# NVlabs/CenterPose

Hardware: NVIDIA H100
Metric: images/sec at 512x512 DLA-34 (dla_34 + DCNv2, 7 heads, decode + PnP) (higher is better)
Workload: dtype tf32x3

## Files before the change

### centerpose_b200/_lib.py

```python
import ctypes
import os

HERE = os.path.dirname(os.path.abspath(__file__))
LIB_PATH = os.environ.get("CP_LIB_PATH") or os.path.join(HERE, "libcenterpose_b200.so")

CP_MAX_HEADS = 16
CP_POSE_RECORD = 192
CP_DETS_RECORD = 128
CP_META_DOUBLES = 16
CP_MAX_K = 128
CP_MAX_MODELS = 16

CP_ARCH_DLA34 = 0
CP_ARCH_DLAV1_34 = 1
CP_ARCH_RES_18, CP_ARCH_RES_34, CP_ARCH_RES_50, CP_ARCH_RES_101, CP_ARCH_RES_152 = 2, 3, 4, 5, 6
CP_PREC_FP32 = 0
CP_PREC_TF32X3 = 1
CP_PREC_BF16 = 2
CP_PREC_TF32 = 3
PRECISIONS = {"fp32": CP_PREC_FP32, "tf32x3": CP_PREC_TF32X3, "bf16": CP_PREC_BF16, "tf32": CP_PREC_TF32}

P_SCORE, P_CLS, P_STATUS, P_NPTS, P_BBOX, P_CT, P_KPS = 0, 1, 2, 3, 4, 8, 10
P_KPS_DISP_MEAN, P_KPS_HM_MEAN, P_KPS_HM_STD, P_KPS_HM_HEIGHT, P_KPS_DISP_STD = 26, 42, 58, 74, 82
P_OBJ_SCALE, P_OBJ_SCALE_UNC, P_TRACKING, P_TRACKING_HP = 98, 101, 104, 106
P_LOCATION, P_QUAT, P_REPROJ, P_PROJ_CUBOID, P_KPS_3D_CAM, P_KPS_PNP, P_SRC_INDEX = 122, 125, 129, 130, 146, 173, 191
D_BBOX, D_SCORE, D_CLS, D_KPS, D_OBJ_SCALE, D_OBJ_SCALE_UNC, D_TRACKING, D_TRACKING_HP = 0, 4, 5, 6, 22, 25, 28, 30
D_KPS_DISP_MEAN, D_KPS_DISP_STD, D_KPS_HM_MEAN, D_KPS_HM_STD, D_KPS_HM_HEIGHT, D_IND = 46, 62, 78, 94, 110, 118
CP_TRACK_RECORD = 320
T_ID, T_AGE, T_ACTIVE, T_IN_BOXES, T_PNP2_STATUS, T_CONF_AVG = 192, 193, 194, 195, 196, 197
T_KPS_FUSION_MEAN, T_KPS_FUSION_STD, T_KPS_MEAN_KF, T_KPS_STD_KF = 200, 216, 232, 248
T_OBJ_SCALE_KF, T_OBJ_SCALE_UNC_KF, T_KPS_PNP_KF, T_KPS_3D_CAM_KF = 264, 267, 270, 288
CP_SEED_RECORD = 264
S_KPS_FUSION_MEAN, S_KPS_FUSION_STD, S_KPS_GT, S_HAS_CT, S_HAS_KPS_GT, S_KPS_PNP_KF, S_HAS_KPS_PNP_KF = 192, 208, 224, 242, 243, 244, 262
RENDER_TRACKS, RENDER_GT, RENDER_EMPTY = 0, 1, 2
PNP_NOT_RUN, PNP_OK, PNP_INVISIBLE, PNP_BEHIND, PNP_FEW_POINTS, PNP_SOLVER_FAIL = 0, 1, 2, 3, 4, 5

EXPORTS = [
    "cp_version", "cp_last_error", "cp_plan_create", "cp_plan_destroy", "cp_plan_load_weights",
    "cp_forward", "cp_plan_bytes", "cp_plan_forward_launches", "cp_decode_workspace_bytes",
    "cp_decode_pnp", "cp_infer", "cp_dcn_v2_forward", "cp_preprocess", "cp_plan_num_ops", "cp_plan_profile",
    "cp_dcn_v2_forward_ex", "cp_conv2d", "cp_dcn_v2_backward",
    "cp_preprocess_affine", "cp_tracker_create", "cp_tracker_destroy", "cp_tracker_reset", "cp_tracker_step", "cp_tracker_render",
    "cp_tracker_render_ex", "cp_tracker_seed", "cp_plan_op_desc", "cp_plan_arena", "cp_plan_run_ops",
    "cp_preprocess_ragged", "cp_tracker_step_ex", "cp_tracker_render_ex2", "cp_tracker_seed_ex",
    "cp_plan_create_multi", "cp_plan_load_weights_model", "cp_plan_num_models", "cp_plan_op_desc_model", "cp_infer_multi",
    "cp_plan_create_multi_track", "cp_infer_multi_track", "cp_tracker_create_multi",
    "cp_plan_create_ex", "cp_plan_memory", "cp_plan_allocations", "cp_preprocess_yuv420",
]

CP_PIX_NV12, CP_PIX_I420 = 0, 1
PIXEL_FORMATS = ("bgr", "nv12", "i420")

CP_PLAN_REUSE_ACTIVATIONS = 1
CP_PLAN_MULTI_TRACK = 2

FAM_NONE, FAM_IGEMM_FP32, FAM_STEM, FAM_CONV3_C16, FAM_IGEMM_UMMA, FAM_CONV_TMA, FAM_DCN_TMA = 0, 1, 2, 3, 4, 5, 6
FAM_MAXPOOL, FAM_UPADD, FAM_GN_RELU, FAM_GRU = 7, 8, 9, 10
FAMILY_NAMES = {FAM_NONE: "fused", FAM_IGEMM_FP32: "igemm_fp32", FAM_STEM: "stem", FAM_CONV3_C16: "conv3_c16",
                FAM_IGEMM_UMMA: "igemm_umma", FAM_CONV_TMA: "conv_tma", FAM_DCN_TMA: "dcn_tma", FAM_MAXPOOL: "maxpool",
                FAM_UPADD: "upadd", FAM_GN_RELU: "gn_relu", FAM_GRU: "gru"}


class CpOpStat(ctypes.Structure):
    _fields_ = [("name", ctypes.c_char * 96), ("kind", ctypes.c_int32), ("ms", ctypes.c_float),
                ("flops", ctypes.c_double), ("bytes", ctypes.c_double)]


class CpActDesc(ctypes.Structure):
    _fields_ = [("off", ctypes.c_int64), ("ext", ctypes.c_int32), ("C", ctypes.c_int32), ("H", ctypes.c_int32),
                ("W", ctypes.c_int32), ("stride", ctypes.c_int32)]


class CpOpDesc(ctypes.Structure):
    _fields_ = ([("name", ctypes.c_char * 96)] +
                [(n, ctypes.c_int32) for n in ("kind", "family", "x3", "nsrc")] +
                [("src", CpActDesc * 4), ("out", CpActDesc), ("out_head", ctypes.c_int32)] +
                [(n, ctypes.c_int32) for n in ("kh", "stride", "pad", "Cin", "Cout", "CoutPad", "Kpad")] +
                [("w", ctypes.c_void_p), ("w_ld", ctypes.c_int32), ("bias", ctypes.c_void_p)] +
                [(n, ctypes.c_int32) for n in ("relu", "has_res", "res_after_relu")] +
                [("res", CpActDesc), ("om", CpActDesc), ("up_w", ctypes.c_void_p), ("f", ctypes.c_int32),
                 ("has_skip", ctypes.c_int32), ("skip", CpActDesc), ("gamma", ctypes.c_void_p),
                 ("beta", ctypes.c_void_p), ("groups", ctypes.c_int32), ("gx", CpActDesc), ("gh", CpActDesc),
                 ("gprev", CpActDesc), ("first_step", ctypes.c_int32)] +
                [(n, ctypes.c_int32) for n in ("fuse_heads", "fused_away", "parent", "n_children")] +
                [("children", ctypes.c_int32 * CP_MAX_HEADS)])


class CpOpLaunch(ctypes.Structure):
    _fields_ = [(n, ctypes.c_int32) for n in ("family", "BN", "ksplit", "grid")]


class CpMemoryInfo(ctypes.Structure):
    _fields_ = [(n, ctypes.c_int64) for n in ("activation_bytes", "weight_bytes", "tile_bytes", "workspace_bytes")]


class CpActAlloc(ctypes.Structure):
    _fields_ = [("floats", ctypes.c_int64), ("off", ctypes.c_int64), ("first", ctypes.c_int32), ("last", ctypes.c_int32)]


class CpConfig(ctypes.Structure):
    _fields_ = [
        ("arch", ctypes.c_int32), ("tracking", ctypes.c_int32), ("tracking_task_gru", ctypes.c_int32),
        ("max_batch", ctypes.c_int32), ("height", ctypes.c_int32), ("width", ctypes.c_int32),
        ("precision", ctypes.c_int32), ("device", ctypes.c_int32), ("head_conv", ctypes.c_int32),
        ("num_heads", ctypes.c_int32),
        ("head_names", ctypes.c_char_p * CP_MAX_HEADS),
        ("head_channels", ctypes.c_int32 * CP_MAX_HEADS),
    ]


class CpHeads(ctypes.Structure):
    _fields_ = [(n, ctypes.c_void_p) for n in (
        "hm", "wh", "hps", "reg", "hm_hp", "hp_offset", "scale", "hps_uncertainty",
        "scale_uncertainty", "tracking", "tracking_hp")]


class CpDecodeParams(ctypes.Structure):
    _fields_ = [
        ("batch", ctypes.c_int32), ("out_h", ctypes.c_int32), ("out_w", ctypes.c_int32),
        ("num_classes", ctypes.c_int32), ("num_joints", ctypes.c_int32), ("K", ctypes.c_int32),
        ("rep_mode", ctypes.c_int32), ("use_moments", ctypes.c_int32), ("nms", ctypes.c_int32),
        ("visible_thresh", ctypes.c_int32), ("opencv_return", ctypes.c_int32),
        ("apply_sigmoid", ctypes.c_int32), ("use_pnp", ctypes.c_int32),
        ("vis_thresh", ctypes.c_float), ("balance", ctypes.c_float), ("modern_bool_semantics", ctypes.c_int32),
        ("test_scale", ctypes.c_float), ("num_scales", ctypes.c_int32),
    ]


class CpTrackerConfig(ctypes.Structure):
    _fields_ = [(n, ctypes.c_int32) for n in (
        "streams", "max_tracks", "kalman", "scale_pool", "use_pnp", "hps_uncertainty", "max_age", "visible_thresh",
        "opencv_return", "render_hm_mode", "render_hmhp_mode", "device")] + [
        (n, ctypes.c_float) for n in ("new_thresh", "pre_thresh", "R", "conf_lo", "conf_hi")] + [
        ("hungarian", ctypes.c_int32)]


_lib = None


def lib_available():
    return os.path.exists(LIB_PATH)


def load():
    global _lib
    if _lib is not None:
        return _lib
    if not os.path.exists(LIB_PATH):
        raise RuntimeError(
            "centerpose_b200: %s not found -- run `python -m centerpose_b200.build` "
            "(there is no CPU / PyTorch fallback for the hot path)" % LIB_PATH)
    L = ctypes.CDLL(LIB_PATH)
    vp, i32, i64 = ctypes.c_void_p, ctypes.c_int32, ctypes.c_int64
    L.cp_version.restype = ctypes.c_int
    L.cp_last_error.restype = ctypes.c_char_p
    L.cp_plan_create.argtypes = [ctypes.POINTER(CpConfig), ctypes.POINTER(vp)]
    L.cp_plan_destroy.argtypes = [vp]
    L.cp_plan_load_weights.argtypes = [vp, ctypes.POINTER(ctypes.c_char_p), ctypes.POINTER(vp),
                                       ctypes.POINTER(i64), i32, vp]
    L.cp_forward.argtypes = [vp, i32, vp, vp, vp, vp, ctypes.POINTER(vp), vp]
    L.cp_plan_num_ops.argtypes = [vp]
    L.cp_plan_profile.argtypes = [vp, i32, vp, vp, vp, vp, ctypes.POINTER(vp), vp, ctypes.POINTER(CpOpStat), i32,
                                  ctypes.POINTER(i32)]
    L.cp_plan_op_desc.argtypes = [vp, i32, ctypes.POINTER(CpOpDesc)]
    L.cp_plan_arena.argtypes = [vp, ctypes.POINTER(vp), ctypes.POINTER(i64)]
    L.cp_plan_run_ops.argtypes = [vp, i32, i32, i32, vp, vp, vp, vp, ctypes.POINTER(vp), vp, ctypes.POINTER(CpOpLaunch)]
    L.cp_plan_bytes.argtypes = [vp]
    L.cp_plan_bytes.restype = i64
    L.cp_plan_forward_launches.argtypes = [vp]
    L.cp_plan_forward_launches.restype = i32
    L.cp_decode_workspace_bytes.argtypes = [ctypes.POINTER(CpDecodeParams)]
    L.cp_decode_workspace_bytes.restype = ctypes.c_size_t
    L.cp_decode_pnp.argtypes = [ctypes.POINTER(CpDecodeParams), ctypes.POINTER(CpHeads), vp, vp, vp, vp, vp,
                                ctypes.c_size_t, vp]
    L.cp_infer.argtypes = [vp, i32, vp, vp, vp, vp, ctypes.POINTER(CpDecodeParams), vp,
                           ctypes.POINTER(vp), vp, vp, vp, vp]
    L.cp_dcn_v2_forward.argtypes = [vp, vp, vp, vp, vp, vp, i32, i32, i32, i32, i32, vp]
    L.cp_dcn_v2_forward_ex.argtypes = [vp, vp, vp, vp, vp, vp, i32, i32, i32, i32, i32, i32, vp]
    L.cp_dcn_v2_backward.argtypes = [vp] * 10 + [i32] * 6 + [vp]
    L.cp_conv2d.argtypes = [vp, vp, vp, vp, vp, i32, i32, i32, i32, i32, i32, i32, i32, i32, i32, vp]
    L.cp_preprocess.argtypes = [vp, vp, i32, i32, i32, i32, i32, ctypes.POINTER(ctypes.c_float),
                                ctypes.POINTER(ctypes.c_float), vp]
    L.cp_preprocess_affine.argtypes = [vp, vp, i32, i32, i32, i32, i32, ctypes.POINTER(ctypes.c_double),
                                       ctypes.POINTER(ctypes.c_float), ctypes.POINTER(ctypes.c_float), vp]
    L.cp_preprocess_ragged.argtypes = [vp, i64, ctypes.POINTER(i64), ctypes.POINTER(i32), vp, i32, i32, i32,
                                       ctypes.POINTER(ctypes.c_double), ctypes.POINTER(ctypes.c_float),
                                       ctypes.POINTER(ctypes.c_float), vp]
    L.cp_preprocess_yuv420.argtypes = [vp, i64, ctypes.POINTER(i64), ctypes.POINTER(i32), i32, vp, i32, i32, i32,
                                       ctypes.POINTER(ctypes.c_double), ctypes.POINTER(ctypes.c_float),
                                       ctypes.POINTER(ctypes.c_float), vp]
    L.cp_tracker_create.argtypes = [ctypes.POINTER(CpTrackerConfig), ctypes.POINTER(vp)]
    L.cp_tracker_destroy.argtypes = [vp]
    L.cp_tracker_reset.argtypes = [vp, i32, vp]
    L.cp_tracker_step.argtypes = [vp, i32, vp, vp, i32, vp, vp, vp, vp]
    L.cp_tracker_render.argtypes = [vp, i32, vp, vp, i32, i32, vp, vp, vp]
    L.cp_tracker_render_ex.argtypes = [vp, i32, vp, vp, i32, i32, ctypes.POINTER(i32), vp, vp, vp]
    L.cp_tracker_seed.argtypes = [vp, i32, vp, vp, i32, vp]
    L.cp_tracker_step_ex.argtypes = [vp, i32, ctypes.POINTER(i32), vp, vp, i32, vp, vp, vp, vp]
    L.cp_tracker_render_ex2.argtypes = [vp, i32, ctypes.POINTER(i32), vp, vp, i32, i32, ctypes.POINTER(i32), vp, vp, vp]
    L.cp_tracker_seed_ex.argtypes = [vp, i32, ctypes.POINTER(i32), vp, vp, i32, vp]
    L.cp_plan_create_multi.argtypes = [ctypes.POINTER(CpConfig), i32, ctypes.POINTER(vp)]
    L.cp_plan_load_weights_model.argtypes = [vp, i32, ctypes.POINTER(ctypes.c_char_p), ctypes.POINTER(vp),
                                             ctypes.POINTER(i64), i32, vp]
    L.cp_plan_num_models.argtypes = [vp]
    L.cp_plan_op_desc_model.argtypes = [vp, i32, i32, ctypes.POINTER(CpOpDesc)]
    L.cp_infer_multi.argtypes = [vp, i32, vp, ctypes.POINTER(CpDecodeParams), vp, ctypes.POINTER(vp), vp, vp, vp, vp]
    L.cp_plan_create_multi_track.argtypes = [ctypes.POINTER(CpConfig), i32, ctypes.POINTER(vp)]
    L.cp_infer_multi_track.argtypes = [vp, i32, vp, vp, vp, vp, ctypes.POINTER(CpDecodeParams), vp, ctypes.POINTER(vp), vp,
                                       vp, vp, vp]
    L.cp_tracker_create_multi.argtypes = [ctypes.POINTER(CpTrackerConfig), i32, ctypes.POINTER(vp)]
    L.cp_plan_create_ex.argtypes = [ctypes.POINTER(CpConfig), i32, ctypes.c_uint32, ctypes.POINTER(vp)]
    L.cp_plan_memory.argtypes = [ctypes.POINTER(CpConfig), i32, ctypes.c_uint32, ctypes.POINTER(CpMemoryInfo)]
    L.cp_plan_allocations.argtypes = [ctypes.POINTER(CpConfig), i32, ctypes.c_uint32, ctypes.POINTER(CpActAlloc), i32,
                                      ctypes.POINTER(i32)]
    for name in EXPORTS:
        fn = getattr(L, name)
        if name not in ("cp_version", "cp_last_error", "cp_plan_bytes", "cp_plan_forward_launches",
                        "cp_decode_workspace_bytes"):
            fn.restype = ctypes.c_int
    _lib = L
    return L


def check(rc, what=""):
    if rc != 0:
        msg = load().cp_last_error()
        raise RuntimeError("centerpose_b200 %s failed (%d): %s" % (what, rc, msg.decode() if msg else "?"))
```

### centerpose_b200/csrc/common.cuh

```cuda
#pragma once
#include <cuda_runtime.h>
#include <stdint.h>
#include <stdio.h>
#include <string>

#include "../../include/centerpose_b200.h"

namespace cp {

void set_error(const std::string& msg);
int fail(int code, const std::string& msg);
extern thread_local long long g_launch_counter;

#define CP_CUDA_CHECK(expr)                                                              \
  do {                                                                                   \
    cudaError_t _e = (expr);                                                             \
    if (_e != cudaSuccess)                                                               \
      return ::cp::fail(CP_ERR_CUDA, std::string(#expr) + ": " + cudaGetErrorString(_e)); \
  } while (0)

#define CP_LAUNCH_CHECK(what)                                                            \
  do {                                                                                   \
    cudaError_t _e = cudaGetLastError();                                                 \
    if (_e != cudaSuccess)                                                               \
      return ::cp::fail(CP_ERR_CUDA, std::string(what) + ": " + cudaGetErrorString(_e));  \
    ++::cp::g_launch_counter;                                                            \
  } while (0)

enum IgemmMode {
  IGEMM_NCHW_SCALAR = 0,
  IGEMM_NHWC_VEC = 1,
  IGEMM_DCN = 2,
  IGEMM_DECONV = 3
};
__host__ __device__ __forceinline__ int deconv_dy(int p, int a) { return p ? 1 - a : -a; }
__host__ __device__ __forceinline__ int deconv_ky(int p, int a) { return p ? 2 * a : 1 + 2 * a; }

struct IgemmParams {
  const float* src[4];
  int srcC[4];
  int srcStride[4];
  int nsrc;
  int B, Hin, Win, Cin;
  int Hout, Wout, Cout, CoutPad;
  int kh, kw, stride, pad;
  int Kpad;
  const float* wgt;
  const float* bias;
  const float* residual;
  int resStride;
  int relu;
  int res_after_relu;
  float* out;
  int outStride;
  int out_nchw;
  const float* offmask;
  int omStride;
  int mask_is_logit;
  int mode;
  const void* wgt_umma;
  float* splitk_ws;
  size_t splitk_ws_floats;
  int fuse_n, fuse_hidden;
  const float* fuse_w[16];
  const float* fuse_b[16];
  float* fuse_out[16];
  int fuse_cout[16];
  int ipm;
  long long wstride, tstride;
  unsigned nchw_per_model;
};
inline int model_ipm(const IgemmParams& p) { return p.ipm > 0 ? p.ipm : p.B; }

int launch_igemm_fp32(const IgemmParams& p, cudaStream_t stream);

int decode_pnp_models(const cp_decode_params* prm, int models, const cp_heads* heads, const double* meta, float* dets,
                      float* poses, int32_t* n_valid, void* workspace, size_t workspace_bytes, void* stream);

struct LaunchInfo {
  int BN = 0;
  int ksplit = 1;
  long long grid = 0;
};

bool conv3_c16_supported(const IgemmParams& p);
int launch_conv3_c16(const IgemmParams& p, cudaStream_t stream);
bool stem_supported(const IgemmParams& p);
int launch_stem_conv(const IgemmParams& p, cudaStream_t s);

struct ConvKernel {
  int family = CP_FAM_IGEMM_FP32;
  bool x3 = false;
  bool round_out = false;
  int BN = 0;
  int cslab = 0;
  size_t wbytes = 0;
};
struct ConvPolicy {
  bool small_on_cuda_cores;
  bool dcn_tma;
  bool round_out;
  bool cuda_core_fallback;
};
inline bool known_precision(int32_t precision) {
  return precision == CP_PREC_FP32 || precision == CP_PREC_TF32X3 || precision == CP_PREC_BF16 || precision == CP_PREC_TF32;
}
inline bool gather_x3(int32_t precision) { return precision == CP_PREC_TF32 || precision == CP_PREC_TF32X3; }
ConvKernel select_conv_kernel(const IgemmParams& p, int32_t precision, const ConvPolicy& pol);
struct alignas(64) TmaMaps {
  unsigned char map[4][128];
};
int conv_encode(const ConvKernel& k, const IgemmParams& p, int Bmax, TmaMaps* maps);
int conv_pack(const ConvKernel& k, const IgemmParams& p, int ld, void* tiles, cudaStream_t s);
int conv_launch(const ConvKernel& k, const IgemmParams& p, const TmaMaps* maps, cudaStream_t s, LaunchInfo* info = nullptr);
int run_conv(IgemmParams& p, int32_t precision, const ConvPolicy& pol, cudaStream_t s);

int splitk_factor(long long tiles, int slabs, int num_sms, size_t tile_floats, size_t ws_floats);

bool umma_supported(const IgemmParams& p, int prec);
int umma_tile_n(int CoutPad, int prec);
size_t umma_weight_bytes(int Kreal, int CoutPad, int prec);
int launch_pack_umma_weight(const float* src_k_by_ld, int ld, int Kreal, int Cout, int CoutPad, int prec, void* dst,
                            cudaStream_t s);
int launch_igemm_umma(const IgemmParams& p, int prec, cudaStream_t stream, LaunchInfo* info = nullptr);

int launch_maxpool2(const float* in, float* out, int B, int H, int W, int C, cudaStream_t s);
int launch_maxpool3s2(const float* in, const float* residual, float* out, int B, int H, int W, int C, cudaStream_t s);
int launch_pack_deconv_weight(const float* w_io44, const float* scale, float* out, int Cin, int Cout, int CoutPad, int Kpad,
                              cudaStream_t s);
int launch_upsample_add(const float* in, const float* wgt_kkc, const float* skip, float* out, int B,
                        int Hin, int Win, int C, int f, cudaStream_t s, int ipm = 0, long long wstride = 0);
int launch_pack_conv_weight(const float* w_oihw, const float* scale, float* out, int Cout, int Cin,
                            int kh, int kw, int CoutPad, int Kpad, int ld, int colOff, cudaStream_t s,
                            int CinPad = 0);
int launch_pack_bias(const float* conv_bias, const float* bn_w, const float* bn_b, const float* bn_mean,
                     const float* bn_var, float* scale_out, float* bias_out, int C, int CPad, float eps,
                     cudaStream_t s);
int launch_pack_up_weight(const float* w_c1kk, float* out_kkc, int C, int k, cudaStream_t s);
int launch_nchw_to_nhwc(const float* in, float* out, int B, int C, int H, int W, int outStride,
                        int chanOffset, cudaStream_t s);
int launch_nhwc_to_nchw(const float* in, float* out, int B, int C, int H, int W, int inStride, cudaStream_t s);
constexpr int kGnBlocks = 64, kGnMaxGroups = 64;
inline size_t gn_workspace_doubles(int B) { return (size_t)B * kGnMaxGroups * 2 * (1 + kGnBlocks); }
int launch_group_norm_relu(float* x, const float* gamma, const float* beta, int B, int HW, int C,
                           int stride, int chanOffset, int groups, float eps, double* ws, cudaStream_t s, int ipm = 0,
                           long long wstride = 0);
int launch_gru_gates(const float* xi, const float* hh, const float* hprev, float* hout, int B_HW, int C,
                     int first_step, cudaStream_t s);

constexpr int kX3GroupBlocks = 1;

bool tma_conv_supported(const IgemmParams& p, int x3);
size_t tma_weight_bytes(int Cin, int taps, int CoutPad, int x3);
int tma_tile_n(int CoutPad, int x3);
int tma_cslab(const IgemmParams& p, int x3);
int launch_pack_tma_weight(const float* src_k_by_ld, int ld, int Cin, int taps, int Cout, int CoutPad, int x3, int cslab,
                           int bn, void* dst, cudaStream_t s);
int tma_encode_nhwc_box(const float* base, int C, int W, int H, int B, int strideFloats, int boxC, int boxW, int boxH,
                        int swizzle64, void* map_out );
int tma_conv_encode(const IgemmParams& p, int Bmax, int cslab, void* maps_out );
int launch_conv_tma(const IgemmParams& p, const void* maps, const ConvKernel& k, cudaStream_t stream, LaunchInfo* info);

bool dcn_tma_supported(const IgemmParams& p, int x3);
int dcn_tma_tile_n(int CoutPad, int x3);
int dcn_tma_encode(const IgemmParams& p, int Bmax, void* map_out );
int launch_dcn_tma(const IgemmParams& p, const void* map, const ConvKernel& k, cudaStream_t stream, LaunchInfo* info);

inline int round_up(int x, int m) { return (x + m - 1) / m * m; }
inline int conv_cout_pad(int Cout) { return round_up(Cout, Cout > 32 ? 64 : (Cout > 16 ? 32 : 16)); }

extern thread_local int g_pdl;
#ifdef __CUDACC__
__device__ __forceinline__ void griddep_wait() { asm volatile("griddepcontrol.wait;" ::: "memory"); }
__device__ __forceinline__ void griddep_launch_dependents() { asm volatile("griddepcontrol.launch_dependents;" ::: "memory"); }
template <typename... KArgs, typename... Args>
inline cudaError_t launch_kernel(void (*kern)(KArgs...), dim3 grid, dim3 block, size_t smem, cudaStream_t s, Args&&... args) {
  cudaLaunchConfig_t cfg{};
  cfg.gridDim = grid;
  cfg.blockDim = block;
  cfg.dynamicSmemBytes = smem;
  cfg.stream = s;
  cudaLaunchAttribute attr[1];
  attr[0].id = cudaLaunchAttributeProgrammaticStreamSerialization;
  attr[0].val.programmaticStreamSerializationAllowed = 1;
  cfg.attrs = attr;
  cfg.numAttrs = g_pdl ? 1 : 0;
  return cudaLaunchKernelEx(&cfg, kern, static_cast<KArgs>(args)...);
}
#endif
constexpr size_t kSplitkWsFloats = (size_t)160 * 256 * 128;

constexpr int kMaxDevices = 64;
inline int current_device_slot() {
  int d = 0;
  if (cudaGetDevice(&d) != cudaSuccess || d < 0 || d >= kMaxDevices) d = 0;
  return d;
}
template <typename T, int N = 1>
struct PerDevice {
  T v[kMaxDevices][N] = {};
  T& here(int slot = 0) { return v[current_device_slot()][slot]; }
};
inline int device_sm_count(int* out) {
  static PerDevice<int> cache;
  int& n = cache.here();
  if (!n) {
    int dev = 0;
    CP_CUDA_CHECK(cudaGetDevice(&dev));
    CP_CUDA_CHECK(cudaDeviceGetAttribute(&n, cudaDevAttrMultiProcessorCount, dev));
  }
  *out = n;
  return CP_OK;
}

}
```

### centerpose_b200/csrc/conv_select.cu

```cuda
#include <stdlib.h>

#include "common.cuh"

namespace cp {

ConvKernel select_conv_kernel(const IgemmParams& p, int32_t precision, const ConvPolicy& pol) {
  const bool small = p.mode == IGEMM_NCHW_SCALAR || p.Cin < 32;
  if (precision != CP_PREC_FP32 && !(pol.small_on_cuda_cores && small)) {
    const bool tma = precision == CP_PREC_TF32 || precision == CP_PREC_TF32X3;
    const bool x3 = precision == CP_PREC_TF32X3;
    if (tma && pol.dcn_tma && dcn_tma_supported(p, x3))
      return {CP_FAM_DCN_TMA, x3, pol.round_out && !x3, dcn_tma_tile_n(p.CoutPad, x3), 16,
              tma_weight_bytes(p.Cin, 9, p.CoutPad, x3)};
    if (tma && tma_conv_supported(p, x3))
      return {CP_FAM_CONV_TMA, x3, pol.round_out && !x3, tma_tile_n(p.CoutPad, x3), tma_cslab(p, x3),
              tma_weight_bytes(p.Cin, p.kh * p.kw, p.CoutPad, x3)};
    const bool gx3 = gather_x3(precision);
    const int phases = p.mode == IGEMM_DECONV ? 4 : 1;
    if (umma_supported(p, gx3))
      return {CP_FAM_IGEMM_UMMA, gx3, false, umma_tile_n(p.CoutPad, gx3), 0,
              phases * umma_weight_bytes(p.kh * p.kw * p.Cin, p.CoutPad, gx3)};
    if (!pol.cuda_core_fallback) return {CP_FAM_NONE};
  }
  return {stem_supported(p) ? CP_FAM_STEM : (conv3_c16_supported(p) ? CP_FAM_CONV3_C16 : CP_FAM_IGEMM_FP32)};
}

int conv_encode(const ConvKernel& k, const IgemmParams& p, int Bmax, TmaMaps* maps) {
  if (k.family == CP_FAM_DCN_TMA) return dcn_tma_encode(p, Bmax, maps->map);
  if (k.family == CP_FAM_CONV_TMA) return tma_conv_encode(p, Bmax, k.cslab, maps->map);
  return CP_OK;
}

int conv_pack(const ConvKernel& k, const IgemmParams& p, int ld, void* tiles, cudaStream_t s) {
  switch (k.family) {
    case CP_FAM_DCN_TMA:
    case CP_FAM_CONV_TMA:
      return launch_pack_tma_weight(p.wgt, ld, p.Cin, p.kh * p.kw, p.Cout, p.CoutPad, k.x3, k.cslab, k.BN, tiles, s);
    case CP_FAM_IGEMM_UMMA: {
      const int phases = p.mode == IGEMM_DECONV ? 4 : 1;
      const size_t phase_bytes = k.wbytes / phases;
      for (int ph = 0; ph < phases; ++ph)
        if (int rc = launch_pack_umma_weight(p.wgt + (size_t)ph * p.Kpad * ld, ld, p.kh * p.kw * p.Cin, p.Cout, p.CoutPad,
                                             k.x3, (unsigned char*)tiles + ph * phase_bytes, s))
          return rc;
      return CP_OK;
    }
    default:
      return CP_OK;
  }
}

int conv_launch(const ConvKernel& k, const IgemmParams& p, const TmaMaps* maps, cudaStream_t s, LaunchInfo* info) {
  switch (k.family) {
    case CP_FAM_DCN_TMA: return launch_dcn_tma(p, maps->map, k, s, info);
    case CP_FAM_CONV_TMA: return launch_conv_tma(p, maps->map, k, s, info);
    case CP_FAM_IGEMM_UMMA: return launch_igemm_umma(p, k.x3, s, info);
    case CP_FAM_STEM: return launch_stem_conv(p, s);
    case CP_FAM_CONV3_C16: return launch_conv3_c16(p, s);
    case CP_FAM_IGEMM_FP32: return launch_igemm_fp32(p, s);
    default: return fail(CP_ERR_INVALID, "conv: no kernel selected");
  }
}

int run_conv(IgemmParams& p, int32_t precision, const ConvPolicy& pol, cudaStream_t s) {
  const ConvKernel k = select_conv_kernel(p, precision, pol);
  if (k.family == CP_FAM_NONE) return fail(CP_ERR_INVALID, "shape not supported by the wgmma kernel");
  if (!k.wbytes) return conv_launch(k, p, nullptr, s);
  void* tiles = nullptr;
  CP_CUDA_CHECK(cudaMallocAsync(&tiles, k.wbytes, s));
  TmaMaps maps;
  int rc = conv_encode(k, p, p.B, &maps);
  if (!rc) rc = conv_pack(k, p, p.CoutPad, tiles, s);
  if (!rc) {
    p.wgt_umma = tiles;
    rc = conv_launch(k, p, &maps, s);
  }
  cudaFreeAsync(tiles, s);
  return rc;
}

int splitk_factor(long long tiles, int slabs, int num_sms, size_t tile_floats, size_t ws_floats) {
  const char* off = getenv("CP_NO_SPLITK");
  if (!ws_floats || (off && atoi(off) != 0)) return 1;
  int S = 1;
  for (int cand = 2; cand <= slabs; ++cand)
    if (slabs % cand == 0 && tiles * cand <= num_sms && (size_t)tiles * cand * tile_floats <= ws_floats) S = cand;
  return S;
}

}
```

### centerpose_b200/csrc/conv_tma.cu

```cuda
#include <cuda.h>

#include "common.cuh"
#include "umma_common.cuh"

namespace cp {
namespace {

constexpr int TM_BM = 128;
constexpr int TM_THREADS = 384;
constexpr int TM_THREADS_X3 = 512;

struct TmaConvParams {
  CUtensorMap amap[4];
  int nsrc;
  int srcC[4];
  int B, H, W, Cin, Cout, CoutPad, BN;
  int k;
  int tile_m;
  int Wt, boxh;
  int tiles_per_image;
  long long total_tiles;
  long long m_tiles;
  uint32_t slab_bytes, slab_stride;
  int SA, SB;
  const float* bias;
  const float* residual;
  int resStride, relu, res_after_relu;
  float* out;
  int outStride, out_nchw;
  int round_tf32;
  int cslab;
  int x3;
  int group;
  const unsigned char* wtiles;
  int ksplit, sps;
  float* part;
  int fuse, tph;
  const float* fuse_w[16];
  const float* fuse_b[16];
  float* fuse_out[16];
  int fuse_cout[16];
  int ipm;
  long long wstride, tstride, tiles_per_model;
};

using namespace umma;

struct TmaCtl {
  unsigned long long a_full[4], a_empty[4], a_split[4];
  unsigned long long b_full[8], b_empty[8];
};
static_assert(sizeof(TmaCtl) <= 512, "control block");

struct TileGeo {
  int n_tile, img, g0, r_lo, model;
  long long pos0;
};
template <bool MULTI>
__device__ __forceinline__ TileGeo decode_tile(const TmaConvParams& p, long long ct, int n_tiles) {
  TileGeo g;
  g.n_tile = (int)(ct % n_tiles);
  const long long m_tile = ct / n_tiles;
  g.img = 0;
  g.g0 = 0;
  g.r_lo = 0;
  g.pos0 = 0;
  g.model = 0;
  if (p.k == 3) {
    g.img = (int)(m_tile / p.tiles_per_image);
    g.g0 = (int)(m_tile - (long long)g.img * p.tiles_per_image) * p.tile_m;
    const int t = g.g0 - 1;
    g.r_lo = (t >= 0) ? t / p.Wt : -((-t + p.Wt - 1) / p.Wt);
    if (MULTI) g.model = g.img / p.ipm;
  } else if (MULTI) {
    g.model = (int)(m_tile / p.tiles_per_model);
    g.pos0 = (long long)g.model * p.ipm * p.H * p.W + (m_tile - g.model * p.tiles_per_model) * p.tile_m;
  } else {
    g.pos0 = m_tile * p.tile_m;
  }
  return g;
}

template <bool MULTI>
__device__ __forceinline__ bool tile_position(const TmaConvParams& p, const TileGeo& g, int i, int* n, int* oy, int* ox, int* m) {
  bool valid;
  if (p.k == 3) {
    const int gg = g.g0 + i;
    *oy = gg / p.Wt;
    const int xp = gg - *oy * p.Wt;
    *ox = xp - 1;
    *n = g.img;
    valid = (*oy < p.H) && (xp >= 1) && (xp <= p.W);
  } else {
    const long long pix = g.pos0 + i;
    valid = pix < (MULTI ? (long long)(g.model + 1) * p.ipm : (long long)p.B) * p.H * p.W;
    const long long pp = valid ? pix : 0;
    *ox = (int)(pp % p.W);
    const long long t = pp / p.W;
    *oy = (int)(t % p.H);
    *n = (int)(t / p.H);
  }
  *m = (int)(((size_t)*n * p.H + *oy) * p.W + *ox);
  return valid;
}

template <bool X3, bool FUSE, int BN, bool MULTI>
__global__ void __launch_bounds__(X3 ? TM_THREADS_X3 : TM_THREADS, 1) conv_tma_kernel(const __grid_constant__ TmaConvParams p) {
  extern __shared__ __align__(1024) unsigned char smem[];
  TmaCtl* ctl = reinterpret_cast<TmaCtl*>(smem);
  if (threadIdx.x == 0) griddep_launch_dependents();
  const uint32_t slabs0 = (smem_u32(smem) + 512u + 1023u) & ~1023u;
  const uint32_t rowb = (uint32_t)p.cslab * 4u;
  const uint32_t btile_bytes = (uint32_t)BN * rowb * (X3 ? 2u : 1u);
  const uint32_t a_stage = p.slab_stride * (X3 ? 2u : 1u);
  const uint32_t btiles0 = slabs0 + (uint32_t)p.SA * a_stage;
  const uint32_t drain0 = btiles0 + (uint32_t)p.SB * btile_bytes;

  const int tid = threadIdx.x, warp = tid >> 5, lane = tid & 31;
  const int n_tiles = p.CoutPad / BN;
  const int taps = p.k * p.k;
  const int KS_SPLIT = p.ksplit;
  const int sps = p.sps;
  const int KB = sps * taps;
  const int KB_all = (p.Cin / p.cslab) * taps;
  const long long total_tiles = p.total_tiles;
  const long long tph = FUSE ? p.tph : 1;
  auto tile_at = [&](long long it) { return ((long long)blockIdx.x + (it / tph) * gridDim.x) * tph + (it % tph); };

  if (tid == 0) {
    for (int s = 0; s < p.SA; ++s) {
      mbar_init(smem_u32(&ctl->a_full[s]), 1);
      mbar_init(smem_u32(&ctl->a_empty[s]), 2);
      mbar_init(smem_u32(&ctl->a_split[s]), 128);
    }
    for (int s = 0; s < p.SB; ++s) {
      mbar_init(smem_u32(&ctl->b_full[s]), 1);
      mbar_init(smem_u32(&ctl->b_empty[s]), 2);
    }
    fence_mbar_init();
  }
  __syncthreads();
  if (warp != 1) griddep_wait();

  if (warp < 4) {
    if (X3) asm volatile("setmaxnreg.dec.sync.aligned.u32 40;");
    if (warp == 0) {
      if (lane == 0) {
        int stage = 0;
        uint32_t phase = 0;
        for (long long it = 0, tile = tile_at(0); tile < total_tiles; tile = tile_at(++it)) {
          const TileGeo g = decode_tile<MULTI>(p, tile / KS_SPLIT, n_tiles);
          const int s_begin = (int)(tile % KS_SPLIT) * sps;
          for (int s = s_begin; s < s_begin + sps; ++s) {
            int src = 0, cb = 0;
            while (src + 1 < p.nsrc && s * p.cslab >= cb + p.srcC[src]) {
              cb += p.srcC[src];
              ++src;
            }
            mbar_wait(smem_u32(&ctl->a_empty[stage]), phase ^ 1u);
            const uint32_t bar = smem_u32(&ctl->a_full[stage]);
            mbar_arrive_expect_tx(bar, p.slab_bytes);
            const uint32_t dst = slabs0 + (uint32_t)stage * a_stage;
            if (p.k == 3)
              tma_load_4d(dst, &p.amap[src], s * p.cslab - cb, -1, g.r_lo - 1, g.img, bar);
            else
              tma_load_2d(dst, &p.amap[src], s * p.cslab - cb, (int)g.pos0, bar);
            if (++stage == p.SA) {
              stage = 0;
              phase ^= 1u;
            }
          }
        }
      }
      __syncwarp();
    } else if (warp == 1) {
      if (lane == 0) {
        int stage = 0;
        uint32_t phase = 0;
        for (long long it = 0, tile = tile_at(0); tile < total_tiles; tile = tile_at(++it)) {
          const unsigned char* wsrc;
          if constexpr (MULTI) {
            const TileGeo g = decode_tile<MULTI>(p, tile / KS_SPLIT, n_tiles);
            wsrc = p.wtiles + (size_t)g.model * p.tstride +
                   ((size_t)g.n_tile * KB_all + (size_t)(tile % KS_SPLIT) * KB) * btile_bytes;
          } else {
            const int n_tile = (int)((tile / KS_SPLIT) % n_tiles);
            wsrc = p.wtiles + ((size_t)n_tile * KB_all + (size_t)(tile % KS_SPLIT) * KB) * btile_bytes;
          }
          for (int kb = 0; kb < KB; ++kb) {
            mbar_wait(smem_u32(&ctl->b_empty[stage]), phase ^ 1u);
            const uint32_t bar = smem_u32(&ctl->b_full[stage]);
            mbar_arrive_expect_tx(bar, btile_bytes);
            bulk_g2s(btiles0 + (uint32_t)stage * btile_bytes, wsrc + (size_t)kb * btile_bytes, btile_bytes, bar);
            if (++stage == p.SB) {
              stage = 0;
              phase ^= 1u;
            }
          }
        }
      }
      __syncwarp();
    }
  } else if (X3 && warp >= 12) {
    asm volatile("setmaxnreg.dec.sync.aligned.u32 48;");
    const int st = tid - 384;
    int stage = 0;
    uint32_t phase = 0;
    const uint32_t nchunk = p.slab_bytes >> 4;
    for (long long it = 0, tile = tile_at(0); tile < total_tiles; tile = tile_at(++it)) {
      for (int s = 0; s < sps; ++s) {
        mbar_wait(smem_u32(&ctl->a_full[stage]), phase);
        const uint32_t hi = slabs0 + (uint32_t)stage * a_stage;
        const uint32_t lo = hi + p.slab_stride;
        for (uint32_t c0 = st; c0 < nchunk; c0 += 128 * 4) {
          float4 v[4];
#pragma unroll
          for (int u = 0; u < 4; ++u)
            if (c0 + u * 128 < nchunk) v[u] = ld_shared_v4f(hi + ((c0 + u * 128) << 4));
#pragma unroll
          for (int u = 0; u < 4; ++u) {
            if (c0 + u * 128 < nchunk) {
              float4 h, l;
              h.x = tf32_round(v[u].x); l.x = tf32_round(v[u].x - h.x);
              h.y = tf32_round(v[u].y); l.y = tf32_round(v[u].y - h.y);
              h.z = tf32_round(v[u].z); l.z = tf32_round(v[u].z - h.z);
              h.w = tf32_round(v[u].w); l.w = tf32_round(v[u].w - h.w);
              st_shared_v4f(hi + ((c0 + u * 128) << 4), h.x, h.y, h.z, h.w);
              st_shared_v4f(lo + ((c0 + u * 128) << 4), l.x, l.y, l.z, l.w);
            }
          }
        }
        fence_proxy_async_smem();
        mbar_arrive(smem_u32(&ctl->a_split[stage]));
        if (++stage == p.SA) {
          stage = 0;
          phase ^= 1u;
        }
      }
    }
  } else {
    if (X3) asm volatile("setmaxnreg.inc.sync.aligned.u32 208;");
    const int c = (warp - 4) >> 2, wt = tid & 127;
    float* dstage = reinterpret_cast<float*>(smem + (drain0 - smem_u32(smem))) + (size_t)c * (DRAIN_STAGE_BYTES / 4);
    const uint32_t bar_a = smem_u32(X3 ? &ctl->a_split[0] : &ctl->a_full[0]);
    const uint32_t bar_a_empty = smem_u32(&ctl->a_empty[0]);
    const uint32_t bar_b_full = smem_u32(&ctl->b_full[0]), bar_b_empty = smem_u32(&ctl->b_empty[0]);
    const uint32_t a_lo_u = p.slab_stride >> 4, b_lo_u = ((uint32_t)BN * rowb) >> 4;
    EpiParams ep;
    ep.bias = p.bias;
    ep.residual = p.residual;
    ep.resStride = p.resStride;
    ep.relu = p.relu;
    ep.res_after_relu = p.res_after_relu;
    ep.round_tf32 = p.round_tf32;
    ep.out = p.out;
    ep.outStride = p.outStride;
    ep.out_nchw = p.out_nchw;
    ep.Cout = p.Cout;
    ep.CoutPad = p.CoutPad;
    ep.H = p.H;
    ep.W = p.W;
    int sa = 0, sb = 0;
    uint32_t pa = 0, pb = 0;
    float acc[BN / 2];
    float sums[X3 ? BN / 2 : 1];
    float acc2[FUSE ? 16 : 1];
#pragma unroll
    for (int j = 0; j < BN / 2; ++j) acc[j] = 0.f;
#pragma unroll
    for (int j = 0; j < (FUSE ? 16 : 1); ++j) acc2[j] = 0.f;
    for (long long it = 0, tile = tile_at(0); tile < total_tiles; tile = tile_at(++it)) {
      const TileGeo g = decode_tile<MULTI>(p, tile / KS_SPLIT, n_tiles);
      const uint32_t row0 = (p.k == 3 ? (uint32_t)(g.g0 - 1 - g.r_lo * p.Wt) : 0u) + (uint32_t)c * 64u;
#pragma unroll
      for (int j = 0; j < (X3 ? BN / 2 : 1); ++j) sums[j] = 0.f;
      int kbi = 0, gk = 0;
      for (int s = 0; s < sps; ++s) {
        mbar_wait(bar_a + 8u * (uint32_t)sa, pa);
        const uint32_t a_slab = slabs0 + (uint32_t)sa * a_stage;
        for (int tap = 0; tap < taps; ++tap, ++kbi) {
          const int ky = tap / 3, kx = tap - ky * 3;
          const uint32_t arow = row0 + (p.k == 3 ? (uint32_t)(ky * p.Wt + kx) : 0u);
          mbar_wait(bar_b_full + 8u * (uint32_t)sb, pb);
          const uint64_t da = make_desc(a_slab + arow * rowb, p.cslab);
          const uint64_t db = make_desc(btiles0 + (uint32_t)sb * btile_bytes, p.cslab);
          const bool fresh = X3 ? gk == 0 : kbi == 0;
          if (p.cslab == 32)
            mma_kblock<BN, X3, false, 4>(acc, da, db, a_lo_u, b_lo_u, fresh);
          else
            mma_kblock<BN, X3, false, 2>(acc, da, db, a_lo_u, b_lo_u, fresh);
          if (wt == 0) {
            mbar_arrive(bar_b_empty + 8u * (uint32_t)sb);
            if (tap == taps - 1) mbar_arrive(bar_a_empty + 8u * (uint32_t)sa);
          }
          if (++sb == p.SB) {
            sb = 0;
            pb ^= 1u;
          }
          if (X3) {
            if (gk == p.group - 1 || kbi == KB - 1) {
#pragma unroll
              for (int j = 0; j < (X3 ? BN / 2 : 1); ++j) sums[j] += acc[X3 ? j : 0];
              gk = 0;
            } else {
              ++gk;
            }
          }
        }
        if (++sa == p.SA) {
          sa = 0;
          pa ^= 1u;
        }
      }
      const int r_me = wt >> 1;
      int n, oy, ox, m;
      const bool valid = tile_position<MULTI>(p, g, c * 64 + r_me, &n, &oy, &ox, &m);
      const int col_end = min(p.Cout, (g.n_tile + 1) * BN);
      const int head = FUSE ? g.n_tile / p.tph : 0, part = FUSE ? g.n_tile - head * p.tph : 0;
      const size_t wofs = MULTI ? (size_t)g.model * p.wstride : 0;
      if (MULTI) ep.bias = p.bias + wofs;
      if (FUSE && part == 0) {
#pragma unroll
        for (int j = 0; j < (FUSE ? 16 : 1); ++j) acc2[j] = 0.f;
      }
      auto fn = [&](int r, int cb, float (&v)[16]) {
        if (cb >= BN) return;
        if (!FUSE && KS_SPLIT > 1) {
          const long long mn = tile / KS_SPLIT;
          const int ks = (int)(tile % KS_SPLIT);
          float4* mine = reinterpret_cast<float4*>(p.part) + (((size_t)mn * KS_SPLIT + ks) * (BN >> 2) + (cb >> 2)) * p.tile_m +
                         c * 64 + r;
#pragma unroll
          for (int q = 0; q < 4; ++q) __stcg(mine + (size_t)q * p.tile_m, make_float4(v[4 * q], v[4 * q + 1], v[4 * q + 2], v[4 * q + 3]));
        } else if (FUSE) {
          const float* b1 = p.bias + wofs + (size_t)g.n_tile * BN + cb;
          const float4* w2 = reinterpret_cast<const float4*>(p.fuse_w[head] + wofs) + ((size_t)part * BN + cb) * 4;
#pragma unroll
          for (int q = 0; q < 16; ++q) {
            const float h = fmaxf(v[q] + __ldg(b1 + q), 0.f);
#pragma unroll
            for (int u = 0; u < 4; ++u) {
              const float4 w = __ldg(w2 + q * 4 + u);
              acc2[FUSE ? 4 * u + 0 : 0] = fmaf(h, w.x, acc2[FUSE ? 4 * u + 0 : 0]);
              acc2[FUSE ? 4 * u + 1 : 0] = fmaf(h, w.y, acc2[FUSE ? 4 * u + 1 : 0]);
              acc2[FUSE ? 4 * u + 2 : 0] = fmaf(h, w.z, acc2[FUSE ? 4 * u + 2 : 0]);
              acc2[FUSE ? 4 * u + 3 : 0] = fmaf(h, w.w, acc2[FUSE ? 4 * u + 3 : 0]);
            }
          }
        } else {
          epilogue_row<16>(ep, v, valid, m, n, oy, ox, g.n_tile * BN + cb, col_end);
        }
      };
      if constexpr (X3)
        drain_rows<BN>(sums, dstage, wt, 1 + c, fn);
      else
        drain_rows<BN>(acc, dstage, wt, 1 + c, fn);
      if (FUSE && part == p.tph - 1) {
#pragma unroll
        for (int j = 0; j < (FUSE ? 16 : 1); ++j) acc2[j] += __shfl_xor_sync(0xffffffffu, acc2[j], 1);
        if ((wt & 1) == 0 && valid) {
          const int co = p.fuse_cout[head];
          float* o = p.fuse_out[head] + ((size_t)n * co * p.H + oy) * p.W + ox;
          const size_t plane = (size_t)p.H * p.W;
#pragma unroll
          for (int j = 0; j < 16; ++j)
            if (j < co) o[j * plane] = acc2[FUSE ? j : 0] + __ldg(p.fuse_b[head] + wofs + j);
        }
      }
    }
  }
}

__global__ void pack_tma_weight_kernel(const float* __restrict__ src, int ld, int Cin, int taps, int Cout, int BN, int n_tiles,
                                       int round_tf32, int x3, int cslab, unsigned char* __restrict__ dst) {
  const int KB = (Cin / cslab) * taps;
  const int cpr = cslab / 4;
  const size_t rowb = (size_t)cslab * 4;
  const size_t total = (size_t)n_tiles * KB * BN * cpr;
  for (size_t i = blockIdx.x * (size_t)blockDim.x + threadIdx.x; i < total; i += (size_t)gridDim.x * blockDim.x) {
    const int q = i % cpr;
    size_t t = i / cpr;
    const int nr = t % BN;
    t /= BN;
    const int kb = t % KB;
    const int nt = t / KB;
    const int n = nt * BN + nr;
    const int slab = kb / taps, tap = kb - slab * taps;
    float v[4];
#pragma unroll
    for (int j = 0; j < 4; ++j) {
      const int k = tap * Cin + slab * cslab + q * 4 + j;
      float x = (n < Cout) ? src[(size_t)k * ld + n] : 0.f;
      v[j] = round_tf32 ? tf32_round(x) : x;
    }
    const size_t tile = ((size_t)nt * KB + kb) * (size_t)BN * rowb * (x3 ? 2 : 1);
    const int sw = cslab == 32 ? (nr & 7) : ((nr >> 1) & 3);
    const size_t off = (size_t)nr * rowb + (size_t)((q ^ sw) << 4);
    *reinterpret_cast<float4*>(dst + tile + off) = make_float4(v[0], v[1], v[2], v[3]);
    if (x3) {
      float l[4];
#pragma unroll
      for (int j = 0; j < 4; ++j) {
        const int k = tap * Cin + slab * cslab + q * 4 + j;
        const float x = (n < Cout) ? src[(size_t)k * ld + n] : 0.f;
        l[j] = tf32_round(x - v[j]);
      }
      *reinterpret_cast<float4*>(dst + tile + (size_t)BN * rowb + off) = make_float4(l[0], l[1], l[2], l[3]);
    }
  }
}

typedef CUresult (*EncodeTiledFn)(CUtensorMap*, CUtensorMapDataType, cuuint32_t, void*, const cuuint64_t*, const cuuint64_t*,
                                  const cuuint32_t*, const cuuint32_t*, CUtensorMapInterleave, CUtensorMapSwizzle,
                                  CUtensorMapL2promotion, CUtensorMapFloatOOBfill);

EncodeTiledFn get_encode() {
  static EncodeTiledFn fn = nullptr;
  if (!fn) {
    void* p = nullptr;
    cudaDriverEntryPointQueryResult q;
    if (cudaGetDriverEntryPoint("cuTensorMapEncodeTiled", &p, cudaEnableDefault, &q) == cudaSuccess &&
        q == cudaDriverEntryPointSuccess)
      fn = (EncodeTiledFn)p;
  }
  return fn;
}

}

template <bool MULTI>
__global__ void __launch_bounds__(256) conv_tma_splitk_finish(const __grid_constant__ TmaConvParams p, long long mn_tiles) {
  splitk_finish<MULTI>(p, p.tile_m, mn_tiles, [&](long long mn, int i, int* n, int* oy, int* ox) {
    int m;
    return tile_position<MULTI>(p, decode_tile<MULTI>(p, mn, p.CoutPad / p.BN), i, n, oy, ox, &m);
  });
}

static int tma_boxh(int Wt) { return (TM_BM + 1 + 2 * Wt + Wt - 1) / Wt + 1; }

constexpr size_t TM_BUDGET = 222 * 1024 - 2 * (size_t)DRAIN_STAGE_BYTES;

static int tma_smem_layout(uint32_t a_stage, uint32_t btile, int k, int* SA, int* SB, size_t* smem) {
  const size_t budget = TM_BUDGET;
  int sa = 2;
  if ((size_t)sa * a_stage + 2 * (size_t)btile > budget) sa = 1;
  if ((size_t)sa * a_stage + 2 * (size_t)btile > budget) return fail(CP_ERR_INVALID, "conv_tma: slab does not fit shared memory");
  int sb = (int)((budget - (size_t)sa * a_stage) / btile);
  if (sb > 8) sb = 8;
  if (sb < 2) return fail(CP_ERR_INVALID, "conv_tma: tile does not fit shared memory");
  if (k == 1 && sa < 4) {
    int s4 = (int)((budget - (size_t)sb * btile) / a_stage);
    if (s4 > 4) s4 = 4;
    if (s4 > sa) sa = s4;
  }
  *SA = sa;
  *SB = sb;
  *smem = 512 + 2048 + (size_t)sa * a_stage + (size_t)sb * btile + 2 * (size_t)DRAIN_STAGE_BYTES;
  return CP_OK;
}

int tma_cslab(const IgemmParams& p, int x3) {
  if (p.Cin % 32) return 16;
  if (!x3 || p.kh != 3) return 32;
  const int Wt = p.Win + 2;
  const int boxh = tma_boxh(Wt);
  const size_t slab32 = ((size_t)boxh * Wt * 128 + 1023) / 1024 * 1024;
  const int bn = tma_tile_n(p.CoutPad, x3);
  const size_t need = 2 * (2 * slab32) + 2 * ((size_t)bn * 128 * 2);
  return need > TM_BUDGET ? 16 : 32;
}

int tma_tile_n(int CoutPad, int) { return wgmma_tile_n(CoutPad, 128); }

bool tma_conv_supported(const IgemmParams& p, int x3) {
  if (p.mode != IGEMM_NHWC_VEC) return false;
  if (!((p.kh == 1 && p.kw == 1 && p.pad == 0) || (p.kh == 3 && p.kw == 3 && p.pad == 1))) return false;
  if (p.stride != 1) return false;
  const int cs = tma_cslab(p, x3);
  if (p.Cin % cs) return false;
  for (int s = 0; s < p.nsrc; ++s)
    if (p.srcC[s] % cs || p.srcStride[s] % 4) return false;
  if (p.kh == 3 && p.Win + 2 > 256) return false;
  const int bn = tma_tile_n(p.CoutPad, x3);
  if (bn == 0) return false;
  const size_t slab = p.kh == 3 ? (size_t)tma_boxh(p.Win + 2) * (p.Win + 2) * cs * 4 : (size_t)TM_BM * cs * 4;
  const size_t a_stage = ((slab + 1023) / 1024 * 1024) * (x3 ? 2 : 1);
  const size_t btile = (size_t)bn * cs * 4 * (x3 ? 2 : 1);
  return a_stage + 2 * btile <= TM_BUDGET;
}

size_t tma_weight_bytes(int Cin, int taps, int CoutPad, int x3) {
  return (size_t)CoutPad * Cin * taps * 4 * (x3 ? 2 : 1);
}

int launch_pack_tma_weight(const float* src, int ld, int Cin, int taps, int Cout, int CoutPad, int x3, int cs, int bn,
                           void* dst, cudaStream_t s) {
  const int nt = CoutPad / bn;
  size_t total = (size_t)nt * (Cin / cs) * taps * bn * (cs / 4);
  int blocks = (int)((total + 255) / 256);
  if (blocks > 132 * 32) blocks = 132 * 32;
  pack_tma_weight_kernel<<<blocks, 256, 0, s>>>(src, ld, Cin, taps, Cout, bn, nt, 1, x3, cs, (unsigned char*)dst);
  CP_LAUNCH_CHECK("pack_tma_weight_kernel");
  return CP_OK;
}

int tma_encode_nhwc_box(const float* base, int C, int W, int H, int B, int strideFloats, int boxC, int boxW, int boxH,
                        int swizzle64, void* map_out) {
  EncodeTiledFn enc = get_encode();
  if (!enc) return fail(CP_ERR_CUDA, "cuTensorMapEncodeTiled entry point not available");
  cuuint64_t dims[4] = {(cuuint64_t)C, (cuuint64_t)W, (cuuint64_t)H, (cuuint64_t)B};
  cuuint64_t strides[3] = {(cuuint64_t)strideFloats * 4, (cuuint64_t)W * strideFloats * 4, (cuuint64_t)H * W * strideFloats * 4};
  cuuint32_t box[4] = {(cuuint32_t)boxC, (cuuint32_t)boxW, (cuuint32_t)boxH, 1};
  cuuint32_t es[4] = {1, 1, 1, 1};
  CUresult r = enc(reinterpret_cast<CUtensorMap*>(map_out), CU_TENSOR_MAP_DATA_TYPE_FLOAT32, 4, (void*)base, dims, strides, box,
                   es, CU_TENSOR_MAP_INTERLEAVE_NONE, swizzle64 ? CU_TENSOR_MAP_SWIZZLE_64B : CU_TENSOR_MAP_SWIZZLE_NONE,
                   CU_TENSOR_MAP_L2_PROMOTION_L2_256B,
                   CU_TENSOR_MAP_FLOAT_OOB_FILL_NONE);
  if (r != CUDA_SUCCESS) return fail(CP_ERR_CUDA, "cuTensorMapEncodeTiled failed with code " + std::to_string((int)r));
  return CP_OK;
}

int tma_conv_encode(const IgemmParams& p, int Bmax, int cs, void* maps_out) {
  EncodeTiledFn enc = get_encode();
  if (!enc) return fail(CP_ERR_CUDA, "cuTensorMapEncodeTiled entry point not available");
  CUtensorMap* maps = reinterpret_cast<CUtensorMap*>(maps_out);
  const int Wt = p.Win + 2;
  const int boxh = tma_boxh(Wt);
  const CUtensorMapSwizzle swz = cs == 32 ? CU_TENSOR_MAP_SWIZZLE_128B : CU_TENSOR_MAP_SWIZZLE_64B;
  for (int s = 0; s < p.nsrc; ++s) {
    CUresult r;
    if (p.kh == 3) {
      cuuint64_t dims[4] = {(cuuint64_t)p.srcC[s], (cuuint64_t)p.Win, (cuuint64_t)p.Hin, (cuuint64_t)Bmax};
      cuuint64_t strides[3] = {(cuuint64_t)p.srcStride[s] * 4, (cuuint64_t)p.Win * p.srcStride[s] * 4,
                               (cuuint64_t)p.Hin * p.Win * p.srcStride[s] * 4};
      cuuint32_t box[4] = {(cuuint32_t)cs, (cuuint32_t)Wt, (cuuint32_t)boxh, 1};
      cuuint32_t es[4] = {1, 1, 1, 1};
      r = enc(&maps[s], CU_TENSOR_MAP_DATA_TYPE_FLOAT32, 4, (void*)p.src[s], dims, strides, box, es,
              CU_TENSOR_MAP_INTERLEAVE_NONE, swz, CU_TENSOR_MAP_L2_PROMOTION_L2_256B,
              CU_TENSOR_MAP_FLOAT_OOB_FILL_NONE);
    } else {
      cuuint64_t dims[2] = {(cuuint64_t)p.srcC[s], (cuuint64_t)Bmax * p.Hin * p.Win};
      cuuint64_t strides[1] = {(cuuint64_t)p.srcStride[s] * 4};
      cuuint32_t box[2] = {(cuuint32_t)cs, (cuuint32_t)TM_BM};
      cuuint32_t es[2] = {1, 1};
      r = enc(&maps[s], CU_TENSOR_MAP_DATA_TYPE_FLOAT32, 2, (void*)p.src[s], dims, strides, box, es,
              CU_TENSOR_MAP_INTERLEAVE_NONE, swz, CU_TENSOR_MAP_L2_PROMOTION_L2_256B,
              CU_TENSOR_MAP_FLOAT_OOB_FILL_NONE);
    }
    if (r != CUDA_SUCCESS) return fail(CP_ERR_CUDA, "cuTensorMapEncodeTiled failed with code " + std::to_string((int)r));
  }
  return CP_OK;
}

template <bool X3, bool FUSE, bool MULTI>
static int launch_conv_tma_kernel(const TmaConvParams& q, const cudaLaunchConfig_t& cfg0) {
  void (*kern)(TmaConvParams) = nullptr;
  switch (q.BN) {
    case 16: kern = conv_tma_kernel<X3, FUSE, 16, MULTI>; break;
    case 32: kern = conv_tma_kernel<X3, FUSE, 32, MULTI>; break;
    case 64: kern = conv_tma_kernel<X3, FUSE, 64, MULTI>; break;
    case 128: kern = conv_tma_kernel<X3, FUSE, 128, MULTI>; break;
    default: return fail(CP_ERR_INVALID, "conv_tma: unsupported N tile");
  }
  static PerDevice<bool, 4> configured;
  const int slot = q.BN == 128 ? 3 : (q.BN == 64 ? 2 : (q.BN == 32 ? 1 : 0));
  if (!configured.here(slot)) {
    CP_CUDA_CHECK(cudaFuncSetAttribute(kern, cudaFuncAttributeMaxDynamicSharedMemorySize, 227 * 1024));
    configured.here(slot) = true;
  }
  cudaLaunchConfig_t cfg = cfg0;
  cudaLaunchAttribute attr[1];
  attr[0].id = cudaLaunchAttributeProgrammaticStreamSerialization;
  attr[0].val.programmaticStreamSerializationAllowed = 1;
  cfg.attrs = attr;
  cfg.numAttrs = g_pdl ? 1 : 0;
  CP_CUDA_CHECK(cudaLaunchKernelEx(&cfg, kern, q));
  CP_LAUNCH_CHECK("conv_tma_kernel");
  return CP_OK;
}

int launch_conv_tma(const IgemmParams& p, const void* maps, const ConvKernel& k, cudaStream_t stream, LaunchInfo* info) {
  if (!p.wgt_umma) return fail(CP_ERR_INVALID, "conv_tma: weight tiles missing");
  if (p.B % model_ipm(p)) return fail(CP_ERR_INVALID, "conv_tma: batch is not a whole number of models");
  const bool x3 = k.x3;
  TmaConvParams q;
  memset(&q, 0, sizeof(q));
  memcpy(q.amap, maps, sizeof(CUtensorMap) * 4);
  q.nsrc = p.nsrc;
  for (int s = 0; s < 4; ++s) q.srcC[s] = p.srcC[s];
  q.B = p.B;
  q.H = p.Hin;
  q.W = p.Win;
  q.Cin = p.Cin;
  q.Cout = p.Cout;
  q.CoutPad = p.CoutPad;
  q.BN = k.BN;
  q.x3 = x3;
  q.cslab = k.cslab;
  q.group = kX3GroupBlocks * (32 / q.cslab);
  q.k = p.kh;
  q.Wt = p.Win + 2;
  q.tile_m = TM_BM;
  q.boxh = tma_boxh(q.Wt);
  q.ipm = model_ipm(p);
  q.wstride = p.wstride;
  q.tstride = p.tstride;
  size_t m_tiles;
  if (q.k == 3) {
    q.tiles_per_image = (p.Hin * q.Wt + q.tile_m - 1) / q.tile_m;
    m_tiles = (size_t)q.tiles_per_image * p.B;
    q.slab_bytes = (uint32_t)q.boxh * q.Wt * (uint32_t)q.cslab * 4u;
  } else {
    q.tiles_per_image = 0;
    q.tiles_per_model = ((long long)q.ipm * p.Hin * p.Win + q.tile_m - 1) / q.tile_m;
    m_tiles = (size_t)q.tiles_per_model * (p.B / q.ipm);
    q.slab_bytes = (uint32_t)q.tile_m * (uint32_t)q.cslab * 4u;
  }
  q.slab_stride = (q.slab_bytes + 1023u) & ~1023u;
  const uint32_t btile = (uint32_t)q.BN * (uint32_t)q.cslab * 4u * (x3 ? 2u : 1u);
  const uint32_t a_stage = q.slab_stride * (x3 ? 2u : 1u);
  size_t smem = 0;
  if (int rc = tma_smem_layout(a_stage, btile, q.k, &q.SA, &q.SB, &smem)) return rc;
  q.bias = p.bias;
  q.residual = p.residual;
  q.resStride = p.resStride;
  q.relu = p.relu;
  q.res_after_relu = p.res_after_relu;
  q.out = p.out;
  q.outStride = p.outStride;
  q.out_nchw = p.out_nchw;
  q.round_tf32 = k.round_out;
  q.wtiles = (const unsigned char*)p.wgt_umma;
  if (p.fuse_n > 0) {
    if (p.fuse_hidden % q.BN || p.CoutPad != p.fuse_n * p.fuse_hidden || !p.relu || p.residual || (x3 && q.BN != 128))
      return fail(CP_ERR_INVALID, "conv_tma: fused 1x1 needs relu, no residual and head_conv a multiple of the N tile");
    q.fuse = 1;
    q.tph = p.fuse_hidden / q.BN;
    for (int h = 0; h < p.fuse_n; ++h) {
      q.fuse_w[h] = p.fuse_w[h];
      q.fuse_b[h] = p.fuse_b[h];
      q.fuse_out[h] = p.fuse_out[h];
      q.fuse_cout[h] = p.fuse_cout[h];
    }
  }
  q.m_tiles = (long long)m_tiles;
  q.part = p.splitk_ws;
  const long long mn = (long long)m_tiles * (p.CoutPad / q.BN);
  const int nslab = q.Cin / q.cslab;
  int num_sms = 0;
  if (int rc = device_sm_count(&num_sms)) return rc;
  q.ksplit = x3 && !q.fuse ? splitk_factor(mn, nslab, num_sms, (size_t)q.tile_m * q.BN, p.splitk_ws_floats) : 1;
  q.sps = nslab / q.ksplit;
  q.total_tiles = mn * q.ksplit;
  if (q.total_tiles >= (1ll << 31)) return fail(CP_ERR_INVALID, "conv_tma: too many tiles");
  cudaLaunchConfig_t cfg{};
  cfg.gridDim = dim3((unsigned)(q.total_tiles < num_sms ? q.total_tiles : num_sms));
  cfg.blockDim = dim3(x3 ? TM_THREADS_X3 : TM_THREADS);
  cfg.dynamicSmemBytes = smem;
  cfg.stream = stream;
  const bool multi = p.B > q.ipm;
  int rc;
  if (multi)
    rc = x3 ? (q.fuse ? launch_conv_tma_kernel<true, true, true>(q, cfg) : launch_conv_tma_kernel<true, false, true>(q, cfg))
            : (q.fuse ? launch_conv_tma_kernel<false, true, true>(q, cfg) : launch_conv_tma_kernel<false, false, true>(q, cfg));
  else
    rc = x3 ? (q.fuse ? launch_conv_tma_kernel<true, true, false>(q, cfg) : launch_conv_tma_kernel<true, false, false>(q, cfg))
            : (q.fuse ? launch_conv_tma_kernel<false, true, false>(q, cfg) : launch_conv_tma_kernel<false, false, false>(q, cfg));
  if (rc) return rc;
  if (info) {
    info->BN = q.BN;
    info->ksplit = q.ksplit;
    info->grid = cfg.gridDim.x;
  }
  if (q.ksplit > 1) {
    const long long threads = mn * (q.BN / 4) * q.tile_m;
    CP_CUDA_CHECK(launch_kernel(multi ? conv_tma_splitk_finish<true> : conv_tma_splitk_finish<false>,
                                dim3((unsigned)((threads + 255) / 256)), dim3(256), 0, stream, q, mn));
    CP_LAUNCH_CHECK("conv_tma_splitk_finish");
  }
  return CP_OK;
}

}
```

### centerpose_b200/csrc/dcn_tma.cu

```cuda
#include <cuda.h>

#include "common.cuh"
#include "umma_common.cuh"

namespace cp {
namespace {

using namespace umma;

constexpr int DT_BM = 128;
constexpr int DT_THREADS = 512;
constexpr int DT_CS = 16;
constexpr int DT_PH = 8, DT_PW = 16;
constexpr int DT_HALO = 8;
constexpr int DT_SH = DT_PH + 2 * DT_HALO, DT_SW = DT_PW + 2 * DT_HALO;
constexpr uint32_t DT_SLAB_BYTES = DT_SH * DT_SW * DT_CS * 4;
constexpr uint32_t DT_COEF_BYTES = DT_BM * 9 * 16;

struct DcnTmaParams {
  CUtensorMap amap;
  const float* src;
  int srcStride;
  const float* offmask;
  int omStride, mask_is_logit;
// ... 341 lines not shown
        if (++sb == p.SB) {
          sb = 0;
          pb ^= 1u;
        }
        if (X3) {
          if (gk == p.group - 1 || kbi == KB - 1) {
#pragma unroll
            for (int j = 0; j < (X3 ? BN / 2 : 1); ++j) sums[j] += acc[X3 ? j : 0];
            gk = 0;
          } else {
            ++gk;
          }
        }
      }
      const int n_tile = (int)((tile / KS_SPLIT) % n_tiles);
      const long long m_tile = (tile / KS_SPLIT) / n_tiles;
      const int n = (int)(m_tile / p.tiles_per_image);
      const int pt = (int)(m_tile - (long long)n * p.tiles_per_image);
      const int col_end = min(p.Cout, (n_tile + 1) * BN);
      if (MULTI) ep.bias = p.bias + (size_t)(n / p.ipm) * p.wstride;
      auto fn = [&](int r, int cb0, float (&v)[16]) {
        if (cb0 >= BN) return;
        const int i = c * 64 + r;
        if (KS_SPLIT > 1) {
          float4* part_row = reinterpret_cast<float4*>(p.part) + ((size_t)tile * (BN >> 2) + (cb0 >> 2)) * 128 + i;
#pragma unroll
          for (int q = 0; q < 4; ++q) __stcg(part_row + (size_t)q * 128, make_float4(v[4 * q], v[4 * q + 1], v[4 * q + 2], v[4 * q + 3]));
        } else {
          const int oy = (pt / p.tiles_x) * DT_PH + (i >> 4), ox = (pt % p.tiles_x) * DT_PW + (i & 15);
          const int m = (n * p.H + oy) * p.W + ox;
          epilogue_row<16>(ep, v, true, m, n, oy, ox, n_tile * BN + cb0, col_end);
        }
      };
      if constexpr (X3)
        drain_rows<BN>(sums, dstage, wt, 1 + c, fn);
      else
        drain_rows<BN>(acc, dstage, wt, 1 + c, fn);
    }
  }
}

template <bool MULTI>
__global__ void __launch_bounds__(256) dcn_tma_splitk_finish(const __grid_constant__ DcnTmaParams p, long long mn_tiles) {
  splitk_finish<MULTI>(p, DT_BM, mn_tiles, [&](long long mn, int i, int* n, int* oy, int* ox) {
    const long long m_tile = mn / (p.CoutPad / p.BN);
    *n = (int)(m_tile / p.tiles_per_image);
    const int pt = (int)(m_tile - (long long)*n * p.tiles_per_image);
    *oy = (pt / p.tiles_x) * DT_PH + (i >> 4);
    *ox = (pt % p.tiles_x) * DT_PW + (i & 15);
    return true;
  });
}

}

int dcn_tma_tile_n(int CoutPad, int) { return wgmma_tile_n(CoutPad, 128); }

bool dcn_tma_supported(const IgemmParams& p, int x3) {
  if (p.mode != IGEMM_DCN || p.nsrc != 1) return false;
  if (p.kh != 3 || p.kw != 3 || p.stride != 1 || p.pad != 1) return false;
  if (p.Cin % DT_CS || p.srcStride[0] % 4) return false;
  const int W = p.Win, H = p.Hin;
  if (W > 128 || H > 128 || (W % DT_PW) || (H % DT_PH)) return false;
  return dcn_tma_tile_n(p.CoutPad, x3) != 0;
}

int dcn_tma_encode(const IgemmParams& p, int Bmax, void* map_out) {
  return tma_encode_nhwc_box(p.src[0], p.srcC[0], p.Win, p.Hin, Bmax, p.srcStride[0], DT_CS, DT_SW, DT_SH, 1, map_out);
}

int launch_dcn_tma(const IgemmParams& p, const void* map, const ConvKernel& k, cudaStream_t stream, LaunchInfo* info) {
  const bool x3 = k.x3;
  if (!p.wgt_umma) return fail(CP_ERR_INVALID, "dcn_tma: weight tiles missing");
  if (!dcn_tma_supported(p, x3)) return fail(CP_ERR_INVALID, "dcn_tma: unsupported shape");
  DcnTmaParams q;
  memset(&q, 0, sizeof(q));
  memcpy(&q.amap, map, sizeof(CUtensorMap));
  q.src = p.src[0];
  q.srcStride = p.srcStride[0];
  q.offmask = p.offmask;
  q.omStride = p.omStride;
  q.mask_is_logit = p.mask_is_logit;
  q.B = p.B;
  q.H = p.Hin;
  q.W = p.Win;
  q.Cin = p.Cin;
  q.Cout = p.Cout;
  q.CoutPad = p.CoutPad;
  q.BN = k.BN;
  q.tiles_x = p.Win / DT_PW;
  q.tiles_per_image = q.tiles_x * (p.Hin / DT_PH);
  const long long mn = (long long)q.tiles_per_image * p.B * (p.CoutPad / q.BN);
  const uint32_t a_stage = 8192u;
  q.group = kX3GroupBlocks * 2;
  const uint32_t btile = (uint32_t)q.BN * 64u * (x3 ? 2u : 1u);
  const size_t budget = 226 * 1024;
  q.AH = 2;
  size_t fixed = 1024 + 2 * (size_t)DT_COEF_BYTES + 1024 + 2 * (size_t)DT_SLAB_BYTES + (size_t)q.AH * a_stage +
                 2 * (size_t)DRAIN_STAGE_BYTES;
  if (fixed + 3 * (size_t)btile > budget) {
    q.AH = 1;
    fixed -= a_stage;
  }
  if (fixed + 2 * (size_t)btile > budget) return fail(CP_ERR_INVALID, "dcn_tma: tile does not fit shared memory");
  q.SB = (int)((budget - fixed) / btile);
  if (q.SB > 8) q.SB = 8;
  q.bias = p.bias;
  q.residual = p.residual;
  q.resStride = p.resStride;
  q.relu = p.relu;
  q.res_after_relu = p.res_after_relu;
  q.out = p.out;
  q.outStride = p.outStride;
  q.out_nchw = p.out_nchw;
  q.round_tf32 = k.round_out;
  q.wtiles = (const unsigned char*)p.wgt_umma;
  q.ipm = model_ipm(p);
  q.wstride = p.wstride;
  q.tstride = p.tstride;
  const bool multi = p.B > q.ipm;
  const size_t smem = fixed + (size_t)q.SB * btile;
  void (*kern)(DcnTmaParams) = nullptr;
  switch (q.BN) {
    case 16: kern = multi ? (x3 ? dcn_tma_kernel<true, 16, true> : dcn_tma_kernel<false, 16, true>)
                          : (x3 ? dcn_tma_kernel<true, 16, false> : dcn_tma_kernel<false, 16, false>); break;
    case 32: kern = multi ? (x3 ? dcn_tma_kernel<true, 32, true> : dcn_tma_kernel<false, 32, true>)
                          : (x3 ? dcn_tma_kernel<true, 32, false> : dcn_tma_kernel<false, 32, false>); break;
    case 64: kern = multi ? (x3 ? dcn_tma_kernel<true, 64, true> : dcn_tma_kernel<false, 64, true>)
                          : (x3 ? dcn_tma_kernel<true, 64, false> : dcn_tma_kernel<false, 64, false>); break;
    case 128: kern = multi ? (x3 ? dcn_tma_kernel<true, 128, true> : dcn_tma_kernel<false, 128, true>)
                           : (x3 ? dcn_tma_kernel<true, 128, false> : dcn_tma_kernel<false, 128, false>); break;
    default: return fail(CP_ERR_INVALID, "dcn_tma: unsupported N tile");
  }
  static PerDevice<bool, 16> configured;
  const int slot = (multi ? 8 : 0) + (x3 ? 4 : 0) + (q.BN == 128 ? 3 : (q.BN == 64 ? 2 : (q.BN == 32 ? 1 : 0)));
  if (!configured.here(slot)) {
    CP_CUDA_CHECK(cudaFuncSetAttribute(kern, cudaFuncAttributeMaxDynamicSharedMemorySize, 227 * 1024));
    configured.here(slot) = true;
  }
  int num_sms = 0;
  if (int rc = device_sm_count(&num_sms)) return rc;
  const int nslab = p.Cin / DT_CS;
  q.part = p.splitk_ws;
  q.ksplit = splitk_factor(mn, nslab, num_sms, (size_t)DT_BM * q.BN, p.splitk_ws_floats);
  q.sps = nslab / q.ksplit;
  q.total_tiles = mn * q.ksplit;
  const unsigned grid = (unsigned)(q.total_tiles < num_sms ? q.total_tiles : num_sms);
  CP_CUDA_CHECK(launch_kernel(kern, dim3(grid), dim3(DT_THREADS), smem, stream, q));
  CP_LAUNCH_CHECK("dcn_tma_kernel");
  if (info) {
    info->BN = q.BN;
    info->ksplit = q.ksplit;
    info->grid = grid;
  }
  if (q.ksplit > 1) {
    const long long threads = mn * (q.BN / 4) * DT_BM;
    CP_CUDA_CHECK(launch_kernel(multi ? dcn_tma_splitk_finish<true> : dcn_tma_splitk_finish<false>, dim3((unsigned)((threads + 255) / 256)), dim3(256), 0, stream, q, mn));
    CP_LAUNCH_CHECK("dcn_tma_splitk_finish");
  }
  return CP_OK;
}

}
```

### centerpose_b200/csrc/plan.cu

```cuda
#include <stdlib.h>
#include <string.h>

#include <map>
#include <memory>
#include <set>
#include <string>
#include <vector>

#include "arena_pack.h"
#include "common.cuh"

namespace cp {

thread_local std::string g_last_error;
void set_error(const std::string& msg) { g_last_error = msg; }
thread_local long long g_launch_counter = 0;
thread_local int g_pdl = 0;

int fail(int code, const std::string& msg) {
  g_last_error = msg;
  return code;
}

namespace {
// ... 842 lines not shown
  cp_plan P;
  if (int rc = plan_layout(&P, cfg, num_models, flags)) return rc;
  const int n = (int)std::min(P.bufs.size(), (size_t)std::max(max_allocs, 0));
  for (int i = 0; i < n; ++i) {
    const ArenaAlloc& b = P.bufs[i];
    const bool mem = !P.reuse || b.first >= 0;
    out[i].floats = mem ? (int64_t)b.floats : 0;
    out[i].off = mem ? (int64_t)P.buf_off[i] : -1;
    out[i].first = b.first;
    out[i].last = b.last;
  }
  *n_allocs = (int32_t)P.bufs.size();
  return CP_OK;
}

int cp_plan_destroy(cp_plan* P) {
  if (!P) return CP_OK;
  cudaFree(P->act);
  cudaFree(P->wts);
  cudaFree(P->gn_stats);
  if (P->umma_wts) cudaFree(P->umma_wts);
  if (P->splitk_ws) cudaFree(P->splitk_ws);
  if (P->decode_ws) cudaFree(P->decode_ws);
  delete P;
  return CP_OK;
}

int64_t cp_plan_bytes(const cp_plan* P) {
  return P ? (int64_t)((P->act_floats + P->w_floats * P->models) * sizeof(float)) : 0;
}
int32_t cp_plan_num_models(const cp_plan* P) { return P ? P->models : 0; }
int32_t cp_plan_forward_launches(const cp_plan* P) { return P ? P->launches : 0; }

int cp_plan_load_weights(cp_plan* P, const char* const* names, const void* const* ptrs, const int64_t* numel,
                         int32_t n, void* stream_) {
  return cp_plan_load_weights_model(P, 0, names, ptrs, numel, n, stream_);
}

int cp_plan_load_weights_model(cp_plan* P, int32_t model, const char* const* names, const void* const* ptrs,
                               const int64_t* numel, int32_t n, void* stream_) {
  if (!P || !names || !ptrs || !numel) return fail(CP_ERR_INVALID, "cp_plan_load_weights: null argument");
  if (model < 0 || model >= P->models) return fail(CP_ERR_INVALID, "cp_plan_load_weights_model: model index out of range");
  cudaStream_t s = (cudaStream_t)stream_;
  float* const wts = P->wts + (size_t)model * P->w_floats;
  std::map<std::string, WRef> m;
  for (int i = 0; i < n; ++i) {
    std::string k = names[i];
    if (k.rfind("module.", 0) == 0 && k.rfind("module_list", 0) != 0) k = k.substr(7);
    m[k] = WRef{(const float*)ptrs[i], numel[i]};
  }
  auto get = [&](const std::string& k, int64_t want, const float** out) -> int {
    auto it = m.find(k);
    if (it == m.end()) return fail(CP_ERR_MISSING_KEY, "state_dict key missing: " + k);
    if (it->second.n != want)
      return fail(CP_ERR_SHAPE, "state_dict key " + k + " has " + std::to_string(it->second.n) + " elements, plan needs " +
                                    std::to_string(want));
    *out = it->second.p;
    return CP_OK;
  };
  int rc;
  for (auto& j : P->jobs) {
    switch (j.type) {
      case PACK_BIAS: {
        const float *cb = nullptr, *g = nullptr, *be = nullptr, *mu = nullptr, *var = nullptr;
        if (!j.key.empty() && (rc = get(j.key, j.Cout, &cb))) return rc;
        if (!j.bn.empty()) {
          if ((rc = get(j.bn + ".weight", j.Cout, &g))) return rc;
          if ((rc = get(j.bn + ".bias", j.Cout, &be))) return rc;
          if ((rc = get(j.bn + ".running_mean", j.Cout, &mu))) return rc;
          if ((rc = get(j.bn + ".running_var", j.Cout, &var))) return rc;
        }
        if ((rc = launch_pack_bias(cb, g, be, mu, var, wts + j.scale, wts + j.dst, j.Cout, j.CoutPad, 1e-5f, s)))
          return rc;
        break;
      }
      case PACK_CONV: {
        const float* w = nullptr;
        if ((rc = get(j.key, (int64_t)j.Cout * j.Cin * j.kh * j.kw, &w))) return rc;
        if ((rc = launch_pack_conv_weight(w, j.use_scale ? wts + j.scale : nullptr, wts + j.dst, j.Cout, j.Cin,
                                          j.kh, j.kw, j.CoutPad, j.Kpad, j.ld, j.colOff, s)))
          return rc;
        break;
      }
      case PACK_UP: {
        const float* w = nullptr;
        if ((rc = get(j.key, (int64_t)j.Cout * j.kh * j.kh, &w))) return rc;
        if ((rc = launch_pack_up_weight(w, wts + j.dst, j.Cout, j.kh, s))) return rc;
        break;
      }
      case PACK_DECONV: {
        const float* w = nullptr;
        if ((rc = get(j.key, (int64_t)j.Cin * j.Cout * 16, &w))) return rc;
        if ((rc = launch_pack_deconv_weight(w, wts + j.scale, wts + j.dst, j.Cin, j.Cout, j.CoutPad, j.Kpad, s))) return rc;
        break;
      }
      case PACK_VEC: {
        const float* w = nullptr;
        if ((rc = get(j.key, j.Cout, &w))) return rc;
        CP_CUDA_CHECK(cudaMemcpyAsync(wts + j.dst, w, sizeof(float) * j.Cout, cudaMemcpyDeviceToDevice, s));
        break;
      }
    }
  }
  for (auto& op : P->ops) {
    if (op.type != OP_IGEMM || !op.kernel.wbytes) continue;
    IgemmParams p;
    plan_params(P, op, &p);
    p.wgt += (size_t)model * P->w_floats;
    if ((rc = conv_pack(op.kernel, p, op.w_ld, P->umma_wts + (size_t)model * P->umma_bytes + op.tile_off, s))) return rc;
  }
  P->model_loaded[model] = 1;
  P->loaded = true;
  for (char l : P->model_loaded) P->loaded = P->loaded && l;
  return CP_OK;
}

struct ProfCtx {
  std::vector<cudaEvent_t> ev;
};

static bool pdl_wanted(long long pixels) {
  if (getenv("CP_NO_PDL")) return false;
  if (const char* e = getenv("CP_PDL")) return atoi(e) != 0;
  return pixels <= 8ll * 512 * 512;
}

static int run_op(cp_plan* P, size_t idx, int batch, const float* const ext[4], float* const* head_out, cudaStream_t s,
                  cp_op_launch* info) {
  int rc;
  const Op& op = P->ops[idx];
  const int images = batch * P->models;
  const long long wstride = (long long)P->w_floats;
  cp_op_launch li{};
  li.ksplit = 1;
  if (op.fused_away) {
    if (info) *info = li;
    return CP_OK;
  }
  switch (op.type) {
    case OP_IGEMM: {
      for (int i = 0; i < op.nsrc; ++i)
        if (op.src[i].ext >= 0 && !ext[op.src[i].ext]) return fail(CP_ERR_INVALID, "cp_forward: a tracking input tensor is null");
      IgemmParams p;
      igemm_params(P, op, batch, ext, head_out, &p);
      p.wgt_umma = P->umma_wts + op.tile_off;
      p.splitk_ws = P->splitk_ws;
      p.splitk_ws_floats = P->splitk_ws ? kSplitkWsFloats : 0;
      LaunchInfo tc;
      li.family = op.kernel.family;
      if ((rc = conv_launch(op.kernel, p, &op.maps, s, &tc))) return rc;
      li.BN = tc.BN;
      li.ksplit = tc.ksplit;
      li.grid = (int32_t)tc.grid;
      break;
    }
    case OP_MAXPOOL:
      li.family = CP_FAM_MAXPOOL;
      if ((rc = launch_maxpool2(P->act + op.src[0].off, P->act + op.out.off, images, op.src[0].H, op.src[0].W,
                                op.src[0].C, s)))
        return rc;
      break;
    case OP_MAXPOOL3:
      li.family = CP_FAM_MAXPOOL;
      if ((rc = launch_maxpool3s2(P->act + op.src[0].off, op.has_res ? P->act + op.res.off : nullptr, P->act + op.out.off,
                                  images, op.src[0].H, op.src[0].W, op.src[0].C, s)))
        return rc;
      break;
    case OP_UPADD:
      li.family = CP_FAM_UPADD;
      if ((rc = launch_upsample_add(P->act + op.src[0].off, P->wts + op.upw_off,
                                    op.has_skip ? P->act + op.skip.off : nullptr, P->act + op.out.off, images,
                                    op.src[0].H, op.src[0].W, op.src[0].C, op.f, s, batch, wstride)))
        return rc;
      break;
    case OP_GN_RELU:
      li.family = CP_FAM_GN_RELU;
      if ((rc = launch_group_norm_relu(P->act + op.out.off, P->wts + op.gamma_off, P->wts + op.beta_off, images,
                                       op.out.H * op.out.W, op.out.C, op.out.stride, 0, op.groups, 1e-5f,
                                       P->gn_stats, s, batch, wstride)))
        return rc;
      break;
    case OP_GRU:
      li.family = CP_FAM_GRU;
      if ((rc = launch_gru_gates(P->act + op.gx.off, op.first_step ? nullptr : P->act + op.gh.off,
                                 op.first_step ? nullptr : P->act + op.gprev.off, P->act + op.out.off,
                                 images * op.out.H * op.out.W, op.out.C, op.first_step, s)))
        return rc;
      break;
  }
  if (info) *info = li;
  return CP_OK;
}

static int run_forward(cp_plan* P, int batch, const float* const ext[4], float* const* head_out, cudaStream_t s,
                       ProfCtx* prof = nullptr) {
  int rc;
  const long long launches0 = g_launch_counter;
  struct PdlScope {
    explicit PdlScope(int on) { g_pdl = on; }
    ~PdlScope() { g_pdl = 0; }
  } pdl_scope(!prof && pdl_wanted((long long)batch * P->models * P->H * P->W));
  for (size_t i = 0; i < P->ops.size(); ++i) {
    if (prof) {
      cudaEvent_t e;
      CP_CUDA_CHECK(cudaEventCreate(&e));
      CP_CUDA_CHECK(cudaEventRecord(e, s));
      prof->ev.push_back(e);
    }
    if ((rc = run_op(P, i, batch, ext, head_out, s, nullptr))) return rc;
  }
  if (prof) {
    cudaEvent_t e;
    CP_CUDA_CHECK(cudaEventCreate(&e));
    CP_CUDA_CHECK(cudaEventRecord(e, s));
    prof->ev.push_back(e);
  }
  P->launches = (int)(g_launch_counter - launches0);
  return CP_OK;
}

static int op_kind(const Op& op) {
  if (op.type == OP_MAXPOOL3) return 11;
  return (int)op.type * 10 + (op.type == OP_IGEMM ? op.mode : 0);
}

static void op_work(const Op& op, int batch, double* flops, double* bytes) {
  *flops = 0;
  *bytes = 0;
  const double B = batch;
  switch (op.type) {
    case OP_IGEMM: {
      int Hin = op.src[0].H, Win = op.src[0].W;
      int Ho = (Hin + 2 * op.pad - op.kh) / op.stride + 1, Wo = (Win + 2 * op.pad - op.kw) / op.stride + 1;
      double M = B * Ho * Wo;
      *flops = 2.0 * M * op.kh * op.kw * op.Cin * op.Cout;
      if (op.mode == IGEMM_DECONV) {
        M = B * op.out.H * op.out.W;
        *flops = 2.0 * M * 4 * op.Cin * op.Cout;
      }
      *bytes = 4.0 * (B * Hin * Win * op.Cin + (double)op.kh * op.kw * op.Cin * op.Cout + (op.fuse_heads ? 0.0 : M * op.Cout) +
                      (op.has_res ? M * op.Cout : 0.0) + (op.mode == IGEMM_DCN ? M * 27 : 0.0));
      if (op.fused_away) {
        *flops = 0;
        *bytes = 0;
      }
      break;
    }
    case OP_MAXPOOL:
      *bytes = 4.0 * B * op.src[0].H * op.src[0].W * op.src[0].C * 1.25;
      break;
    case OP_MAXPOOL3:
      *bytes = 4.0 * B * op.src[0].H * op.src[0].W * op.src[0].C * (op.has_res ? 1.5 : 1.25);
      break;
    case OP_UPADD: {
      double o = B * op.out.H * op.out.W * op.out.C;
      *flops = 2.0 * o * 4;
      *bytes = 4.0 * (o * 2 + B * op.src[0].H * op.src[0].W * op.src[0].C);
      break;
    }
    case OP_GN_RELU:
      *bytes = 4.0 * B * op.out.H * op.out.W * op.out.C * 3;
      break;
    case OP_GRU:
      *bytes = 4.0 * B * op.out.H * op.out.W * op.out.C * 8;
      break;
  }
}

static int check_run(const cp_plan* P, bool given, int32_t batch, const char* fn, const char* load = "cp_plan_load_weights") {
  if (!P || !given) return fail(CP_ERR_INVALID, std::string(fn) + ": null argument");
  if (!P->loaded) return fail(CP_ERR_NOT_LOADED, std::string(fn) + ": call " + load + " first");
  if (batch <= 0 || batch > P->B) return fail(CP_ERR_INVALID, std::string(fn) + ": batch exceeds the plan's max_batch");
  return CP_OK;
}
static const char* const kLoadEveryModel = "cp_plan_load_weights_model for every model";

int cp_forward(cp_plan* P, int32_t batch, const float* images, const float* pre_img, const float* pre_hm,
               const float* pre_hm_hp, float* const* head_out, void* stream) {
  if (int rc = check_run(P, images && head_out, batch, "cp_forward")) return rc;
  const float* ext[4] = {images, pre_img, pre_hm, pre_hm_hp};
  return run_forward(P, batch, ext, head_out, (cudaStream_t)stream);
}

int cp_plan_num_ops(const cp_plan* P) { return P ? (int)P->ops.size() : 0; }

int cp_plan_profile(cp_plan* P, int32_t batch, const float* images, const float* pre_img, const float* pre_hm,
                    const float* pre_hm_hp, float* const* head_out, void* stream, cp_op_stat* stats, int32_t max_stats,
                    int32_t* n_stats) {
  if (int rc = check_run(P, images && head_out && stats && n_stats, batch, "cp_plan_profile")) return rc;
  const float* ext[4] = {images, pre_img, pre_hm, pre_hm_hp};
  ProfCtx ctx;
  int rc = run_forward(P, batch, ext, head_out, (cudaStream_t)stream, &ctx);
  if (rc == CP_OK) {
    CP_CUDA_CHECK(cudaEventSynchronize(ctx.ev.back()));
    int n = 0;
    for (size_t i = 0; i + 1 < ctx.ev.size() && n < max_stats; ++i, ++n) {
      const Op& op = P->ops[i];
      cp_op_stat& st = stats[n];
      memset(&st, 0, sizeof(st));
      snprintf(st.name, sizeof(st.name), "%s", op.name.c_str());
      st.kind = op_kind(op);
      cudaEventElapsedTime(&st.ms, ctx.ev[i], ctx.ev[i + 1]);
      op_work(op, batch * P->models, &st.flops, &st.bytes);
    }
    *n_stats = n;
  }
// ... 209 lines not shown
```

### centerpose_b200/csrc/umma_common.cuh

```cuda
#pragma once
#include <cuda.h>
#include <cuda_runtime.h>
#include <stdint.h>
#include <stdio.h>

namespace cp {
namespace umma {

__device__ __forceinline__ uint32_t smem_u32(const void* p) { return (uint32_t)__cvta_generic_to_shared(p); }

__device__ __forceinline__ void mbar_init(uint32_t bar, uint32_t count) {
  asm volatile("mbarrier.init.shared::cta.b64 [%0], %1;" ::"r"(bar), "r"(count));
}
__device__ __forceinline__ void mbar_arrive(uint32_t bar) {
  asm volatile("mbarrier.arrive.shared::cta.b64 _, [%0];" ::"r"(bar) : "memory");
}
__device__ __forceinline__ void mbar_arrive_expect_tx(uint32_t bar, uint32_t bytes) {
  asm volatile("mbarrier.arrive.expect_tx.shared::cta.b64 _, [%0], %1;" ::"r"(bar), "r"(bytes) : "memory");
}
__device__ __forceinline__ bool mbar_try_wait(uint32_t bar, uint32_t parity) {
  uint32_t ok;
  asm volatile(
      "{\n\t.reg .pred p;\n\tmbarrier.try_wait.parity.shared::cta.b64 p, [%1], %2;\n\tselp.b32 %0, 1, 0, p;\n\t}"
      : "=r"(ok)
      : "r"(bar), "r"(parity)
      : "memory");
  return ok != 0;
}
__device__ __forceinline__ void mbar_wait(uint32_t bar, uint32_t parity) {
  if (mbar_try_wait(bar, parity)) return;
  const long long t0 = clock64();
  while (!mbar_try_wait(bar, parity)) {
    if (clock64() - t0 > 4000000000LL) {
#ifdef CP_MBAR_DEBUG
      printf("wgmma kernel: mbarrier watchdog (block %d thread %d bar %u parity %u)\n", blockIdx.x, threadIdx.x, bar, parity);
#endif
      __trap();
    }
  }
}
__device__ __forceinline__ void fence_proxy_async_smem() { asm volatile("fence.proxy.async.shared::cta;" ::: "memory"); }
__device__ __forceinline__ void fence_mbar_init() { asm volatile("fence.mbarrier_init.release.cluster;" ::: "memory"); }

__device__ __forceinline__ void bulk_g2s(uint32_t dst, const void* src, uint32_t bytes, uint32_t bar) {
  asm volatile("cp.async.bulk.shared::cluster.global.mbarrier::complete_tx::bytes [%0], [%1], %2, [%3];" ::"r"(dst),
               "l"(src), "r"(bytes), "r"(bar)
               : "memory");
}
__device__ __forceinline__ void wg_bar_sync(int id) { asm volatile("bar.sync %0, 128;" ::"r"(id) : "memory"); }

__device__ __forceinline__ void wg_fence() { asm volatile("wgmma.fence.sync.aligned;" ::: "memory"); }
__device__ __forceinline__ void wg_commit() { asm volatile("wgmma.commit_group.sync.aligned;" ::: "memory"); }
template <int N>
__device__ __forceinline__ void wg_wait() { asm volatile("wgmma.wait_group.sync.aligned %0;" ::"n"(N) : "memory"); }
template <int N>
__device__ __forceinline__ void wgmma_tf32(float (&d)[N / 2], uint64_t da, uint64_t db, uint32_t scale_d);
template <int N>
__device__ __forceinline__ void wgmma_bf16(float (&d)[N / 2], uint64_t da, uint64_t db, uint32_t scale_d);
template <> __device__ __forceinline__ void wgmma_tf32<16>(float (&d)[8], uint64_t da, uint64_t db, uint32_t scale_d) {
  asm volatile(
      "{\n\t.reg .pred p;\n\tsetp.ne.b32 p, %10, 0;\n\t"
      "wgmma.mma_async.sync.aligned.m64n16k8.f32.tf32.tf32 {%0,%1,%2,%3,%4,%5,%6,%7}, %8, %9, p, 1, 1;\n\t}"
      : "+f"(d[0]), "+f"(d[1]), "+f"(d[2]), "+f"(d[3]), "+f"(d[4]), "+f"(d[5]), "+f"(d[6]), "+f"(d[7])
      : "l"(da), "l"(db), "r"(scale_d));
}
template <> __device__ __forceinline__ void wgmma_tf32<32>(float (&d)[16], uint64_t da, uint64_t db, uint32_t scale_d) {
  asm volatile(
      "{\n\t.reg .pred p;\n\tsetp.ne.b32 p, %18, 0;\n\t"
      "wgmma.mma_async.sync.aligned.m64n32k8.f32.tf32.tf32 {%0,%1,%2,%3,%4,%5,%6,%7,%8,%9,%10,%11,%12,%13,%14,%15}, %16, %17, p, 1, 1;\n\t}"
      : "+f"(d[0]), "+f"(d[1]), "+f"(d[2]), "+f"(d[3]), "+f"(d[4]), "+f"(d[5]), "+f"(d[6]), "+f"(d[7]), "+f"(d[8]), "+f"(d[9]), "+f"(d[10]), "+f"(d[11]), "+f"(d[12]), "+f"(d[13]), "+f"(d[14]), "+f"(d[15])
      : "l"(da), "l"(db), "r"(scale_d));
}
template <> __device__ __forceinline__ void wgmma_tf32<64>(float (&d)[32], uint64_t da, uint64_t db, uint32_t scale_d) {
  asm volatile(
      "{\n\t.reg .pred p;\n\tsetp.ne.b32 p, %34, 0;\n\t"
      "wgmma.mma_async.sync.aligned.m64n64k8.f32.tf32.tf32 {%0,%1,%2,%3,%4,%5,%6,%7,%8,%9,%10,%11,%12,%13,%14,%15,%16,%17,%18,%19,%20,%21,%22,%23,%24,%25,%26,%27,%28,%29,%30,%31}, %32, %33, p, 1, 1;\n\t}"
      : "+f"(d[0]), "+f"(d[1]), "+f"(d[2]), "+f"(d[3]), "+f"(d[4]), "+f"(d[5]), "+f"(d[6]), "+f"(d[7]), "+f"(d[8]), "+f"(d[9]), "+f"(d[10]), "+f"(d[11]), "+f"(d[12]), "+f"(d[13]), "+f"(d[14]), "+f"(d[15]), "+f"(d[16]), "+f"(d[17]), "+f"(d[18]), "+f"(d[19]), "+f"(d[20]), "+f"(d[21]), "+f"(d[22]), "+f"(d[23]), "+f"(d[24]), "+f"(d[25]), "+f"(d[26]), "+f"(d[27]), "+f"(d[28]), "+f"(d[29]), "+f"(d[30]), "+f"(d[31])
      : "l"(da), "l"(db), "r"(scale_d));
}
template <> __device__ __forceinline__ void wgmma_tf32<128>(float (&d)[64], uint64_t da, uint64_t db, uint32_t scale_d) {
  asm volatile(
      "{\n\t.reg .pred p;\n\tsetp.ne.b32 p, %66, 0;\n\t"
      "wgmma.mma_async.sync.aligned.m64n128k8.f32.tf32.tf32 {%0,%1,%2,%3,%4,%5,%6,%7,%8,%9,%10,%11,%12,%13,%14,%15,%16,%17,%18,%19,%20,%21,%22,%23,%24,%25,%26,%27,%28,%29,%30,%31,%32,%33,%34,%35,%36,%37,%38,%39,%40,%41,%42,%43,%44,%45,%46,%47,%48,%49,%50,%51,%52,%53,%54,%55,%56,%57,%58,%59,%60,%61,%62,%63}, %64, %65, p, 1, 1;\n\t}"
      : "+f"(d[0]), "+f"(d[1]), "+f"(d[2]), "+f"(d[3]), "+f"(d[4]), "+f"(d[5]), "+f"(d[6]), "+f"(d[7]), "+f"(d[8]), "+f"(d[9]), "+f"(d[10]), "+f"(d[11]), "+f"(d[12]), "+f"(d[13]), "+f"(d[14]), "+f"(d[15]), "+f"(d[16]), "+f"(d[17]), "+f"(d[18]), "+f"(d[19]), "+f"(d[20]), "+f"(d[21]), "+f"(d[22]), "+f"(d[23]), "+f"(d[24]), "+f"(d[25]), "+f"(d[26]), "+f"(d[27]), "+f"(d[28]), "+f"(d[29]), "+f"(d[30]), "+f"(d[31]), "+f"(d[32]), "+f"(d[33]), "+f"(d[34]), "+f"(d[35]), "+f"(d[36]), "+f"(d[37]), "+f"(d[38]), "+f"(d[39]), "+f"(d[40]), "+f"(d[41]), "+f"(d[42]), "+f"(d[43]), "+f"(d[44]), "+f"(d[45]), "+f"(d[46]), "+f"(d[47]), "+f"(d[48]), "+f"(d[49]), "+f"(d[50]), "+f"(d[51]), "+f"(d[52]), "+f"(d[53]), "+f"(d[54]), "+f"(d[55]), "+f"(d[56]), "+f"(d[57]), "+f"(d[58]), "+f"(d[59]), "+f"(d[60]), "+f"(d[61]), "+f"(d[62]), "+f"(d[63])
      : "l"(da), "l"(db), "r"(scale_d));
}
template <> __device__ __forceinline__ void wgmma_tf32<256>(float (&d)[128], uint64_t da, uint64_t db, uint32_t scale_d) {
  asm volatile(
      "{\n\t.reg .pred p;\n\tsetp.ne.b32 p, %130, 0;\n\t"
      "wgmma.mma_async.sync.aligned.m64n256k8.f32.tf32.tf32 {%0,%1,%2,%3,%4,%5,%6,%7,%8,%9,%10,%11,%12,%13,%14,%15,%16,%17,%18,%19,%20,%21,%22,%23,%24,%25,%26,%27,%28,%29,%30,%31,%32,%33,%34,%35,%36,%37,%38,%39,%40,%41,%42,%43,%44,%45,%46,%47,%48,%49,%50,%51,%52,%53,%54,%55,%56,%57,%58,%59,%60,%61,%62,%63,%64,%65,%66,%67,%68,%69,%70,%71,%72,%73,%74,%75,%76,%77,%78,%79,%80,%81,%82,%83,%84,%85,%86,%87,%88,%89,%90,%91,%92,%93,%94,%95,%96,%97,%98,%99,%100,%101,%102,%103,%104,%105,%106,%107,%108,%109,%110,%111,%112,%113,%114,%115,%116,%117,%118,%119,%120,%121,%122,%123,%124,%125,%126,%127}, %128, %129, p, 1, 1;\n\t}"
      : "+f"(d[0]), "+f"(d[1]), "+f"(d[2]), "+f"(d[3]), "+f"(d[4]), "+f"(d[5]), "+f"(d[6]), "+f"(d[7]), "+f"(d[8]), "+f"(d[9]), "+f"(d[10]), "+f"(d[11]), "+f"(d[12]), "+f"(d[13]), "+f"(d[14]), "+f"(d[15]), "+f"(d[16]), "+f"(d[17]), "+f"(d[18]), "+f"(d[19]), "+f"(d[20]), "+f"(d[21]), "+f"(d[22]), "+f"(d[23]), "+f"(d[24]), "+f"(d[25]), "+f"(d[26]), "+f"(d[27]), "+f"(d[28]), "+f"(d[29]), "+f"(d[30]), "+f"(d[31]), "+f"(d[32]), "+f"(d[33]), "+f"(d[34]), "+f"(d[35]), "+f"(d[36]), "+f"(d[37]), "+f"(d[38]), "+f"(d[39]), "+f"(d[40]), "+f"(d[41]), "+f"(d[42]), "+f"(d[43]), "+f"(d[44]), "+f"(d[45]), "+f"(d[46]), "+f"(d[47]), "+f"(d[48]), "+f"(d[49]), "+f"(d[50]), "+f"(d[51]), "+f"(d[52]), "+f"(d[53]), "+f"(d[54]), "+f"(d[55]), "+f"(d[56]), "+f"(d[57]), "+f"(d[58]), "+f"(d[59]), "+f"(d[60]), "+f"(d[61]), "+f"(d[62]), "+f"(d[63]), "+f"(d[64]), "+f"(d[65]), "+f"(d[66]), "+f"(d[67]), "+f"(d[68]), "+f"(d[69]), "+f"(d[70]), "+f"(d[71]), "+f"(d[72]), "+f"(d[73]), "+f"(d[74]), "+f"(d[75]), "+f"(d[76]), "+f"(d[77]), "+f"(d[78]), "+f"(d[79]), "+f"(d[80]), "+f"(d[81]), "+f"(d[82]), "+f"(d[83]), "+f"(d[84]), "+f"(d[85]), "+f"(d[86]), "+f"(d[87]), "+f"(d[88]), "+f"(d[89]), "+f"(d[90]), "+f"(d[91]), "+f"(d[92]), "+f"(d[93]), "+f"(d[94]), "+f"(d[95]), "+f"(d[96]), "+f"(d[97]), "+f"(d[98]), "+f"(d[99]), "+f"(d[100]), "+f"(d[101]), "+f"(d[102]), "+f"(d[103]), "+f"(d[104]), "+f"(d[105]), "+f"(d[106]), "+f"(d[107]), "+f"(d[108]), "+f"(d[109]), "+f"(d[110]), "+f"(d[111]), "+f"(d[112]), "+f"(d[113]), "+f"(d[114]), "+f"(d[115]), "+f"(d[116]), "+f"(d[117]), "+f"(d[118]), "+f"(d[119]), "+f"(d[120]), "+f"(d[121]), "+f"(d[122]), "+f"(d[123]), "+f"(d[124]), "+f"(d[125]), "+f"(d[126]), "+f"(d[127])
      : "l"(da), "l"(db), "r"(scale_d));
}
template <> __device__ __forceinline__ void wgmma_bf16<16>(float (&d)[8], uint64_t da, uint64_t db, uint32_t scale_d) {
  asm volatile(
      "{\n\t.reg .pred p;\n\tsetp.ne.b32 p, %10, 0;\n\t"
      "wgmma.mma_async.sync.aligned.m64n16k16.f32.bf16.bf16 {%0,%1,%2,%3,%4,%5,%6,%7}, %8, %9, p, 1, 1, 0, 0;\n\t}"
      : "+f"(d[0]), "+f"(d[1]), "+f"(d[2]), "+f"(d[3]), "+f"(d[4]), "+f"(d[5]), "+f"(d[6]), "+f"(d[7])
      : "l"(da), "l"(db), "r"(scale_d));
}
template <> __device__ __forceinline__ void wgmma_bf16<32>(float (&d)[16], uint64_t da, uint64_t db, uint32_t scale_d) {
  asm volatile(
      "{\n\t.reg .pred p;\n\tsetp.ne.b32 p, %18, 0;\n\t"
      "wgmma.mma_async.sync.aligned.m64n32k16.f32.bf16.bf16 {%0,%1,%2,%3,%4,%5,%6,%7,%8,%9,%10,%11,%12,%13,%14,%15}, %16, %17, p, 1, 1, 0, 0;\n\t}"
      : "+f"(d[0]), "+f"(d[1]), "+f"(d[2]), "+f"(d[3]), "+f"(d[4]), "+f"(d[5]), "+f"(d[6]), "+f"(d[7]), "+f"(d[8]), "+f"(d[9]), "+f"(d[10]), "+f"(d[11]), "+f"(d[12]), "+f"(d[13]), "+f"(d[14]), "+f"(d[15])
      : "l"(da), "l"(db), "r"(scale_d));
}
template <> __device__ __forceinline__ void wgmma_bf16<64>(float (&d)[32], uint64_t da, uint64_t db, uint32_t scale_d) {
  asm volatile(
      "{\n\t.reg .pred p;\n\tsetp.ne.b32 p, %34, 0;\n\t"
      "wgmma.mma_async.sync.aligned.m64n64k16.f32.bf16.bf16 {%0,%1,%2,%3,%4,%5,%6,%7,%8,%9,%10,%11,%12,%13,%14,%15,%16,%17,%18,%19,%20,%21,%22,%23,%24,%25,%26,%27,%28,%29,%30,%31}, %32, %33, p, 1, 1, 0, 0;\n\t}"
      : "+f"(d[0]), "+f"(d[1]), "+f"(d[2]), "+f"(d[3]), "+f"(d[4]), "+f"(d[5]), "+f"(d[6]), "+f"(d[7]), "+f"(d[8]), "+f"(d[9]), "+f"(d[10]), "+f"(d[11]), "+f"(d[12]), "+f"(d[13]), "+f"(d[14]), "+f"(d[15]), "+f"(d[16]), "+f"(d[17]), "+f"(d[18]), "+f"(d[19]), "+f"(d[20]), "+f"(d[21]), "+f"(d[22]), "+f"(d[23]), "+f"(d[24]), "+f"(d[25]), "+f"(d[26]), "+f"(d[27]), "+f"(d[28]), "+f"(d[29]), "+f"(d[30]), "+f"(d[31])
      : "l"(da), "l"(db), "r"(scale_d));
}
template <> __device__ __forceinline__ void wgmma_bf16<128>(float (&d)[64], uint64_t da, uint64_t db, uint32_t scale_d) {
  asm volatile(
      "{\n\t.reg .pred p;\n\tsetp.ne.b32 p, %66, 0;\n\t"
      "wgmma.mma_async.sync.aligned.m64n128k16.f32.bf16.bf16 {%0,%1,%2,%3,%4,%5,%6,%7,%8,%9,%10,%11,%12,%13,%14,%15,%16,%17,%18,%19,%20,%21,%22,%23,%24,%25,%26,%27,%28,%29,%30,%31,%32,%33,%34,%35,%36,%37,%38,%39,%40,%41,%42,%43,%44,%45,%46,%47,%48,%49,%50,%51,%52,%53,%54,%55,%56,%57,%58,%59,%60,%61,%62,%63}, %64, %65, p, 1, 1, 0, 0;\n\t}"
      : "+f"(d[0]), "+f"(d[1]), "+f"(d[2]), "+f"(d[3]), "+f"(d[4]), "+f"(d[5]), "+f"(d[6]), "+f"(d[7]), "+f"(d[8]), "+f"(d[9]), "+f"(d[10]), "+f"(d[11]), "+f"(d[12]), "+f"(d[13]), "+f"(d[14]), "+f"(d[15]), "+f"(d[16]), "+f"(d[17]), "+f"(d[18]), "+f"(d[19]), "+f"(d[20]), "+f"(d[21]), "+f"(d[22]), "+f"(d[23]), "+f"(d[24]), "+f"(d[25]), "+f"(d[26]), "+f"(d[27]), "+f"(d[28]), "+f"(d[29]), "+f"(d[30]), "+f"(d[31]), "+f"(d[32]), "+f"(d[33]), "+f"(d[34]), "+f"(d[35]), "+f"(d[36]), "+f"(d[37]), "+f"(d[38]), "+f"(d[39]), "+f"(d[40]), "+f"(d[41]), "+f"(d[42]), "+f"(d[43]), "+f"(d[44]), "+f"(d[45]), "+f"(d[46]), "+f"(d[47]), "+f"(d[48]), "+f"(d[49]), "+f"(d[50]), "+f"(d[51]), "+f"(d[52]), "+f"(d[53]), "+f"(d[54]), "+f"(d[55]), "+f"(d[56]), "+f"(d[57]), "+f"(d[58]), "+f"(d[59]), "+f"(d[60]), "+f"(d[61]), "+f"(d[62]), "+f"(d[63])
      : "l"(da), "l"(db), "r"(scale_d));
}
template <> __device__ __forceinline__ void wgmma_bf16<256>(float (&d)[128], uint64_t da, uint64_t db, uint32_t scale_d) {
  asm volatile(
      "{\n\t.reg .pred p;\n\tsetp.ne.b32 p, %130, 0;\n\t"
      "wgmma.mma_async.sync.aligned.m64n256k16.f32.bf16.bf16 {%0,%1,%2,%3,%4,%5,%6,%7,%8,%9,%10,%11,%12,%13,%14,%15,%16,%17,%18,%19,%20,%21,%22,%23,%24,%25,%26,%27,%28,%29,%30,%31,%32,%33,%34,%35,%36,%37,%38,%39,%40,%41,%42,%43,%44,%45,%46,%47,%48,%49,%50,%51,%52,%53,%54,%55,%56,%57,%58,%59,%60,%61,%62,%63,%64,%65,%66,%67,%68,%69,%70,%71,%72,%73,%74,%75,%76,%77,%78,%79,%80,%81,%82,%83,%84,%85,%86,%87,%88,%89,%90,%91,%92,%93,%94,%95,%96,%97,%98,%99,%100,%101,%102,%103,%104,%105,%106,%107,%108,%109,%110,%111,%112,%113,%114,%115,%116,%117,%118,%119,%120,%121,%122,%123,%124,%125,%126,%127}, %128, %129, p, 1, 1, 0, 0;\n\t}"
      : "+f"(d[0]), "+f"(d[1]), "+f"(d[2]), "+f"(d[3]), "+f"(d[4]), "+f"(d[5]), "+f"(d[6]), "+f"(d[7]), "+f"(d[8]), "+f"(d[9]), "+f"(d[10]), "+f"(d[11]), "+f"(d[12]), "+f"(d[13]), "+f"(d[14]), "+f"(d[15]), "+f"(d[16]), "+f"(d[17]), "+f"(d[18]), "+f"(d[19]), "+f"(d[20]), "+f"(d[21]), "+f"(d[22]), "+f"(d[23]), "+f"(d[24]), "+f"(d[25]), "+f"(d[26]), "+f"(d[27]), "+f"(d[28]), "+f"(d[29]), "+f"(d[30]), "+f"(d[31]), "+f"(d[32]), "+f"(d[33]), "+f"(d[34]), "+f"(d[35]), "+f"(d[36]), "+f"(d[37]), "+f"(d[38]), "+f"(d[39]), "+f"(d[40]), "+f"(d[41]), "+f"(d[42]), "+f"(d[43]), "+f"(d[44]), "+f"(d[45]), "+f"(d[46]), "+f"(d[47]), "+f"(d[48]), "+f"(d[49]), "+f"(d[50]), "+f"(d[51]), "+f"(d[52]), "+f"(d[53]), "+f"(d[54]), "+f"(d[55]), "+f"(d[56]), "+f"(d[57]), "+f"(d[58]), "+f"(d[59]), "+f"(d[60]), "+f"(d[61]), "+f"(d[62]), "+f"(d[63]), "+f"(d[64]), "+f"(d[65]), "+f"(d[66]), "+f"(d[67]), "+f"(d[68]), "+f"(d[69]), "+f"(d[70]), "+f"(d[71]), "+f"(d[72]), "+f"(d[73]), "+f"(d[74]), "+f"(d[75]), "+f"(d[76]), "+f"(d[77]), "+f"(d[78]), "+f"(d[79]), "+f"(d[80]), "+f"(d[81]), "+f"(d[82]), "+f"(d[83]), "+f"(d[84]), "+f"(d[85]), "+f"(d[86]), "+f"(d[87]), "+f"(d[88]), "+f"(d[89]), "+f"(d[90]), "+f"(d[91]), "+f"(d[92]), "+f"(d[93]), "+f"(d[94]), "+f"(d[95]), "+f"(d[96]), "+f"(d[97]), "+f"(d[98]), "+f"(d[99]), "+f"(d[100]), "+f"(d[101]), "+f"(d[102]), "+f"(d[103]), "+f"(d[104]), "+f"(d[105]), "+f"(d[106]), "+f"(d[107]), "+f"(d[108]), "+f"(d[109]), "+f"(d[110]), "+f"(d[111]), "+f"(d[112]), "+f"(d[113]), "+f"(d[114]), "+f"(d[115]), "+f"(d[116]), "+f"(d[117]), "+f"(d[118]), "+f"(d[119]), "+f"(d[120]), "+f"(d[121]), "+f"(d[122]), "+f"(d[123]), "+f"(d[124]), "+f"(d[125]), "+f"(d[126]), "+f"(d[127])
      : "l"(da), "l"(db), "r"(scale_d));
}

template <int N>
__device__ __forceinline__ void wgmma_tf32_rs(float (&d)[N / 2], const uint32_t (&a)[4], uint64_t db, uint32_t scale_d);
template <> __device__ __forceinline__ void wgmma_tf32_rs<16>(float (&d)[8], const uint32_t (&a)[4], uint64_t db, uint32_t scale_d) {
  asm volatile(
      "{\n\t.reg .pred p;\n\tsetp.ne.b32 p, %13, 0;\n\t"
      "wgmma.mma_async.sync.aligned.m64n16k8.f32.tf32.tf32 {%0,%1,%2,%3,%4,%5,%6,%7}, {%8,%9,%10,%11}, %12, p, 1, 1;\n\t}"
      : "+f"(d[0]), "+f"(d[1]), "+f"(d[2]), "+f"(d[3]), "+f"(d[4]), "+f"(d[5]), "+f"(d[6]), "+f"(d[7])
      : "r"(a[0]), "r"(a[1]), "r"(a[2]), "r"(a[3]), "l"(db), "r"(scale_d));
}
template <> __device__ __forceinline__ void wgmma_tf32_rs<32>(float (&d)[16], const uint32_t (&a)[4], uint64_t db, uint32_t scale_d) {
  asm volatile(
      "{\n\t.reg .pred p;\n\tsetp.ne.b32 p, %21, 0;\n\t"
      "wgmma.mma_async.sync.aligned.m64n32k8.f32.tf32.tf32 {%0,%1,%2,%3,%4,%5,%6,%7,%8,%9,%10,%11,%12,%13,%14,%15}, {%16,%17,%18,%19}, %20, p, 1, 1;\n\t}"
      : "+f"(d[0]), "+f"(d[1]), "+f"(d[2]), "+f"(d[3]), "+f"(d[4]), "+f"(d[5]), "+f"(d[6]), "+f"(d[7]), "+f"(d[8]), "+f"(d[9]), "+f"(d[10]), "+f"(d[11]), "+f"(d[12]), "+f"(d[13]), "+f"(d[14]), "+f"(d[15])
      : "r"(a[0]), "r"(a[1]), "r"(a[2]), "r"(a[3]), "l"(db), "r"(scale_d));
}
template <> __device__ __forceinline__ void wgmma_tf32_rs<64>(float (&d)[32], const uint32_t (&a)[4], uint64_t db, uint32_t scale_d) {
  asm volatile(
      "{\n\t.reg .pred p;\n\tsetp.ne.b32 p, %37, 0;\n\t"
      "wgmma.mma_async.sync.aligned.m64n64k8.f32.tf32.tf32 {%0,%1,%2,%3,%4,%5,%6,%7,%8,%9,%10,%11,%12,%13,%14,%15,%16,%17,%18,%19,%20,%21,%22,%23,%24,%25,%26,%27,%28,%29,%30,%31}, {%32,%33,%34,%35}, %36, p, 1, 1;\n\t}"
      : "+f"(d[0]), "+f"(d[1]), "+f"(d[2]), "+f"(d[3]), "+f"(d[4]), "+f"(d[5]), "+f"(d[6]), "+f"(d[7]), "+f"(d[8]), "+f"(d[9]), "+f"(d[10]), "+f"(d[11]), "+f"(d[12]), "+f"(d[13]), "+f"(d[14]), "+f"(d[15]), "+f"(d[16]), "+f"(d[17]), "+f"(d[18]), "+f"(d[19]), "+f"(d[20]), "+f"(d[21]), "+f"(d[22]), "+f"(d[23]), "+f"(d[24]), "+f"(d[25]), "+f"(d[26]), "+f"(d[27]), "+f"(d[28]), "+f"(d[29]), "+f"(d[30]), "+f"(d[31])
      : "r"(a[0]), "r"(a[1]), "r"(a[2]), "r"(a[3]), "l"(db), "r"(scale_d));
}
template <> __device__ __forceinline__ void wgmma_tf32_rs<128>(float (&d)[64], const uint32_t (&a)[4], uint64_t db, uint32_t scale_d) {
  asm volatile(
      "{\n\t.reg .pred p;\n\tsetp.ne.b32 p, %69, 0;\n\t"
      "wgmma.mma_async.sync.aligned.m64n128k8.f32.tf32.tf32 {%0,%1,%2,%3,%4,%5,%6,%7,%8,%9,%10,%11,%12,%13,%14,%15,%16,%17,%18,%19,%20,%21,%22,%23,%24,%25,%26,%27,%28,%29,%30,%31,%32,%33,%34,%35,%36,%37,%38,%39,%40,%41,%42,%43,%44,%45,%46,%47,%48,%49,%50,%51,%52,%53,%54,%55,%56,%57,%58,%59,%60,%61,%62,%63}, {%64,%65,%66,%67}, %68, p, 1, 1;\n\t}"
      : "+f"(d[0]), "+f"(d[1]), "+f"(d[2]), "+f"(d[3]), "+f"(d[4]), "+f"(d[5]), "+f"(d[6]), "+f"(d[7]), "+f"(d[8]), "+f"(d[9]), "+f"(d[10]), "+f"(d[11]), "+f"(d[12]), "+f"(d[13]), "+f"(d[14]), "+f"(d[15]), "+f"(d[16]), "+f"(d[17]), "+f"(d[18]), "+f"(d[19]), "+f"(d[20]), "+f"(d[21]), "+f"(d[22]), "+f"(d[23]), "+f"(d[24]), "+f"(d[25]), "+f"(d[26]), "+f"(d[27]), "+f"(d[28]), "+f"(d[29]), "+f"(d[30]), "+f"(d[31]), "+f"(d[32]), "+f"(d[33]), "+f"(d[34]), "+f"(d[35]), "+f"(d[36]), "+f"(d[37]), "+f"(d[38]), "+f"(d[39]), "+f"(d[40]), "+f"(d[41]), "+f"(d[42]), "+f"(d[43]), "+f"(d[44]), "+f"(d[45]), "+f"(d[46]), "+f"(d[47]), "+f"(d[48]), "+f"(d[49]), "+f"(d[50]), "+f"(d[51]), "+f"(d[52]), "+f"(d[53]), "+f"(d[54]), "+f"(d[55]), "+f"(d[56]), "+f"(d[57]), "+f"(d[58]), "+f"(d[59]), "+f"(d[60]), "+f"(d[61]), "+f"(d[62]), "+f"(d[63])
      : "r"(a[0]), "r"(a[1]), "r"(a[2]), "r"(a[3]), "l"(db), "r"(scale_d));
}

template <int BN, bool X3, bool BF16, int KS>
__device__ __forceinline__ void mma_kblock(float (&acc)[BN / 2], uint64_t da, uint64_t db, uint32_t a_lo, uint32_t b_lo,
                                           bool fresh) {
  wg_fence();
#pragma unroll
  for (int ks = 0; ks < KS; ++ks) {
    const uint32_t sd = (fresh && ks == 0) ? 0u : 1u;
    if (X3) {
      wgmma_tf32<BN>(acc, da + a_lo + 2u * ks, db + 2u * ks, sd);
      wgmma_tf32<BN>(acc, da + 2u * ks, db + b_lo + 2u * ks, 1u);
    } else if (BF16) {
      wgmma_bf16<BN>(acc, da + 2u * ks, db + 2u * ks, sd);
    } else {
      wgmma_tf32<BN>(acc, da + 2u * ks, db + 2u * ks, sd);
    }
  }
  if (X3) {
#pragma unroll
    for (int ks = 0; ks < KS; ++ks) wgmma_tf32<BN>(acc, da + 2u * ks, db + 2u * ks, 1u);
  }
  wg_commit();
  wg_wait<0>();
}

__device__ __forceinline__ float tf32_round(float x) {
  return __uint_as_float((__float_as_uint(x) + 0x1000u) & 0xffffe000u);
}
__device__ __forceinline__ void ldsm_x4(uint32_t (&r)[4], uint32_t addr) {
  asm volatile("ldmatrix.sync.aligned.m8n8.x4.shared.b16 {%0, %1, %2, %3}, [%4];"
               : "=r"(r[0]), "=r"(r[1]), "=r"(r[2]), "=r"(r[3])
               : "r"(addr));
}

template <int BN, int KS>
__device__ __forceinline__ void mma_kblock_x3(float (&acc)[BN / 2], uint32_t a_tile, int wt, uint64_t db, uint32_t b_lo,
                                              bool fresh) {
  const uint32_t lane = (uint32_t)wt & 31u;
  const uint32_t row = (uint32_t)(wt >> 5) * 16u + (lane & 7u) + ((lane >> 3) & 1u) * 8u;
  const uint32_t a_row = a_tile + row * (32u * KS);
  const uint32_t x = ((lane >> 4) << 4) ^ ((a_row >> 3) & (KS == 4 ? 0x70u : 0x30u));
  uint32_t hi[KS][4], lo[KS][4];
#pragma unroll
  for (int ks = 0; ks < KS; ++ks) {
    ldsm_x4(hi[ks], a_row + (((uint32_t)ks << 5) ^ x));
#pragma unroll
    for (int j = 0; j < 4; ++j) {
      const float v = __uint_as_float(hi[ks][j]);
      const float h = tf32_round(v);
      lo[ks][j] = __float_as_uint(tf32_round(v - h));
      hi[ks][j] = __float_as_uint(h);
    }
  }
  wg_fence();
#pragma unroll
  for (int ks = 0; ks < KS; ++ks) {
    wgmma_tf32_rs<BN>(acc, lo[ks], db + 2u * ks, (fresh && ks == 0) ? 0u : 1u);
    wgmma_tf32_rs<BN>(acc, hi[ks], db + b_lo + 2u * ks, 1u);
  }
#pragma unroll
  for (int ks = 0; ks < KS; ++ks) wgmma_tf32_rs<BN>(acc, hi[ks], db + 2u * ks, 1u);
  wg_commit();
  wg_wait<0>();
#pragma unroll
  for (int ks = 0; ks < KS; ++ks)
#pragma unroll
    for (int j = 0; j < 4; ++j) asm volatile("" : "+r"(hi[ks][j]), "+r"(lo[ks][j]));
}

__device__ __forceinline__ uint32_t pack_bf16x2(float a, float b) {
  uint32_t r;
  asm("cvt.rn.bf16x2.f32 %0, %1, %2;" : "=r"(r) : "f"(b), "f"(a));
  return r;
}
__device__ __forceinline__ void st_shared_v4(uint32_t addr, uint32_t a, uint32_t b, uint32_t c, uint32_t d) {
  asm volatile("st.shared.v4.b32 [%0], {%1, %2, %3, %4};" ::"r"(addr), "r"(a), "r"(b), "r"(c), "r"(d) : "memory");
}
__device__ __forceinline__ void st_shared_v4f(uint32_t addr, float a, float b, float c, float d) {
  asm volatile("st.shared.v4.f32 [%0], {%1, %2, %3, %4};" ::"r"(addr), "f"(a), "f"(b), "f"(c), "f"(d) : "memory");
}
__device__ __forceinline__ float4 ld_shared_v4f(uint32_t addr) {
  float4 v;
  asm volatile("ld.shared.v4.f32 {%0,%1,%2,%3}, [%4];" : "=f"(v.x), "=f"(v.y), "=f"(v.z), "=f"(v.w) : "r"(addr) : "memory");
  return v;
}

__device__ __forceinline__ void tma_load_4d(uint32_t dst, const CUtensorMap* map, int c0, int c1, int c2, int c3, uint32_t bar) {
  asm volatile(
      "cp.async.bulk.tensor.4d.shared::cluster.global.tile.mbarrier::complete_tx::bytes [%0], [%1, {%2, %3, %4, %5}], [%6];" ::"r"(dst),
      "l"(map), "r"(c0), "r"(c1), "r"(c2), "r"(c3), "r"(bar)
      : "memory");
}
__device__ __forceinline__ void tma_load_2d(uint32_t dst, const CUtensorMap* map, int c0, int c1, uint32_t bar) {
  asm volatile("cp.async.bulk.tensor.2d.shared::cluster.global.tile.mbarrier::complete_tx::bytes [%0], [%1, {%2, %3}], [%4];" ::"r"(dst),
               "l"(map), "r"(c0), "r"(c1), "r"(bar)
               : "memory");
}
__device__ __forceinline__ bool elect_one() {
  uint32_t pred;
  asm volatile("{\n\t.reg .pred p;\n\telect.sync _|p, 0xffffffff;\n\tselp.u32 %0, 1, 0, p;\n\t}" : "=r"(pred));
  return pred != 0;
}

__device__ __forceinline__ uint64_t make_desc(uint32_t saddr, int cslab) {
  const uint64_t sbo = cslab == 32 ? (1024 >> 4) : (512 >> 4);
  const uint64_t lay = cslab == 32 ? 1ull : 2ull;
  return (uint64_t)((saddr >> 4) & 0x3FFFu) | (1ull << 16) | (sbo << 32) | (lay << 62);
}

struct EpiParams {
  const float* bias;
  const float* residual;
  int resStride, relu, res_after_relu, round_tf32;
  float* out;
  int outStride, out_nchw;
  int Cout, CoutPad, H, W;
};

template <int NV>
__device__ __forceinline__ void epilogue_row(const EpiParams& e, float (&vv)[NV], bool valid, int m, int n, int oy, int ox,
                                             int col0, int col_end) {
#pragma unroll
  for (int j = 0; j < NV; ++j)
    if (col0 + j < e.CoutPad) vv[j] += __ldg(e.bias + col0 + j);
  if (e.residual && valid && !e.res_after_relu) {
    const float* r = e.residual + (size_t)m * e.resStride + col0;
#pragma unroll
    for (int j = 0; j < NV; ++j)
      if (col0 + j < col_end) vv[j] += __ldg(r + j);
  }
  if (e.relu) {
#pragma unroll
    for (int j = 0; j < NV; ++j) vv[j] = fmaxf(vv[j], 0.f);
  }
  if (e.residual && valid && e.res_after_relu) {
    const float* r = e.residual + (size_t)m * e.resStride + col0;
#pragma unroll
    for (int j = 0; j < NV; ++j)
      if (col0 + j < col_end) vv[j] += __ldg(r + j);
  }
  if (e.round_tf32) {
#pragma unroll
    for (int j = 0; j < NV; ++j) vv[j] = tf32_round(vv[j]);
  }
  if (!valid) return;
  if (e.out_nchw) {
#pragma unroll
    for (int j = 0; j < NV; ++j)
      if (col0 + j < col_end) e.out[(((size_t)n * e.Cout + col0 + j) * e.H + oy) * e.W + ox] = vv[j];
  } else {
    float* o = e.out + (size_t)m * e.outStride + col0;
#pragma unroll
    for (int j = 0; j < NV; j += 4) {
      if (col0 + j + 3 < col_end) {
        *reinterpret_cast<float4*>(o + j) = make_float4(vv[j], vv[j + 1], vv[j + 2], vv[j + 3]);
      } else {
#pragma unroll
        for (int t = 0; t < 4; ++t)
          if (col0 + j + t < col_end) o[j + t] = vv[j + t];
      }
    }
  }
}

template <bool MULTI, class Params, class RowAt>
__device__ __forceinline__ void splitk_finish(const Params& p, int rows, long long mn_tiles, RowAt row_at) {
  griddep_launch_dependents();
  griddep_wait();
  const int G = p.BN >> 2;
  const long long idx = (long long)blockIdx.x * blockDim.x + threadIdx.x;
  if (idx >= mn_tiles * G * rows) return;
  const int i = (int)(idx % rows);
  const int c4 = (int)((idx / rows) % G);
  const long long mn = idx / ((long long)rows * G);
  const float4* src = reinterpret_cast<const float4*>(p.part) + ((size_t)mn * p.ksplit * G + c4) * rows + i;
  float4 a = make_float4(0.f, 0.f, 0.f, 0.f);
// ... 51 lines not shown
```

### centerpose_b200/engine.py

```python
import ctypes

import numpy as np
import torch

from . import _lib

HEAD_FIELDS = ("hm", "wh", "hps", "reg", "hm_hp", "hp_offset", "scale", "hps_uncertainty",
               "scale_uncertainty", "tracking", "tracking_hp")
_VISIBLE = {"book": 6, "chair": 6, "cereal_box": 6, "camera": 3, "bottle": 3, "cup": 3,
            "bike": 0, "laptop": 0, "shoe": 0}


def _ptr(t):
    return ctypes.c_void_p(t.data_ptr()) if t is not None else ctypes.c_void_p(0)


def _stream():
    return ctypes.c_void_p(torch.cuda.current_stream().cuda_stream)


def decode_params(opt=None, **over):
    g = lambda n, d: over.get(n, getattr(opt, n, d) if opt is not None else d)
    p = _lib.CpDecodeParams()
    p.num_classes = int(g("num_classes", 1))
# ... 146 lines not shown
                                   tracking_task_gru, precision)
        self._cfg = cfg
        plan = ctypes.c_void_p()
        flags = _plan_flags(self.tracking, self.models, self.reuse_activations)
        with torch.cuda.device(self.device):
            _lib.check(self.L.cp_plan_create_ex(ctypes.byref(cfg), self.models, flags, ctypes.byref(plan)), "cp_plan_create")
        self.plan = plan
        self.weights_sig = None
        self.forward_launches = int(self.L.cp_plan_forward_launches(plan))
        self.plan_bytes = int(self.L.cp_plan_bytes(plan))
        self.memory = plan_memory(arch, heads, head_conv, max_batch, height, width, tracking, tracking_task_gru, precision,
                                  self.models, self.reuse_activations)

    def close(self):
        if getattr(self, "plan", None):
            self.L.cp_plan_destroy(self.plan)
            self.plan = None

    def __del__(self):
        try:
            self.close()
        except Exception:
            pass

    def load_state_dict(self, sd, model=0):
        names, ptrs, numel, keep = [], [], [], []
        for k, v in sd.items():
            if not torch.is_tensor(v) or not v.dtype.is_floating_point:
                continue
            t = v.detach().to(self.device, torch.float32).contiguous()
            keep.append(t)
            names.append(k.encode())
            ptrs.append(t.data_ptr())
            numel.append(t.numel())
        n = len(names)
        a_names = (ctypes.c_char_p * n)(*names)
        a_ptrs = (ctypes.c_void_p * n)(*ptrs)
        a_numel = (ctypes.c_int64 * n)(*numel)
        with torch.cuda.device(self.device):
            rc = self.L.cp_plan_load_weights_model(self.plan, int(model), a_names, a_ptrs, a_numel, n, _stream())
            _lib.check(rc, "cp_plan_load_weights")
            torch.cuda.current_stream().synchronize()

    def _dev(self, t, name, shape):
        if not torch.is_tensor(t):
            raise TypeError("%s must be a torch tensor" % name)
        if tuple(t.shape) != tuple(shape):
            raise ValueError("%s %s does not fit the plan: expected %s" % (name, tuple(t.shape), tuple(shape)))
        if t.device != self.device or t.dtype != torch.float32:
            t = t.to(self.device, torch.float32)
        return t.contiguous()

    def _check_inputs(self, x, pre_img, pre_hm, pre_hm_hp):
        B = x.shape[0]
        if x.dim() != 4 or tuple(x.shape[1:]) != (3, self.height, self.width) or B > self.max_batch or B < 1:
            raise ValueError("input %s does not fit the plan (%d,3,%d,%d)" % (tuple(x.shape), self.max_batch,
                                                                            self.height, self.width))
        xs = [self._dev(x, "images", (B, 3, self.height, self.width))]
        if self.tracking:
            if pre_img is None or pre_hm is None or pre_hm_hp is None:
                raise ValueError("a tracking plan needs pre_img, pre_hm and pre_hm_hp")
            lead = self._lead(B)
            xs += [self._dev(pre_img, "pre_img", (B, 3, self.height, self.width)),
                   self._dev(pre_hm, "pre_hm", lead + (1, self.height, self.width)),
                   self._dev(pre_hm_hp, "pre_hm_hp", lead + (8, self.height, self.width))]
        else:
            xs += [None, None, None]
        return B, xs

    def _out_tensor(self, t, name, shape, dtype):
        if t.device != self.device or t.dtype != dtype or tuple(t.shape) != tuple(shape) or not t.is_contiguous():
            raise ValueError("%s must be a contiguous %s tensor of shape %s on %s" % (name, dtype, tuple(shape), self.device))
        return t

    def _lead(self, B):
        return (self.models, B) if self.models > 1 else (B,)

    def _head_shape(self, B, c):
        return self._lead(B) + (c, self.height // 4, self.width // 4)

    def forward(self, x, pre_img=None, pre_hm=None, pre_hm_hp=None, out=None):
        B, xs = self._check_inputs(x, pre_img, pre_hm, pre_hm_hp)
        if out is None:
            out = {n: torch.empty(self._head_shape(B, c), dtype=torch.float32, device=self.device)
                   for n, c in self.heads.items()}
        else:
            for n, c in self.heads.items():
                self._out_tensor(out[n], "out[%s]" % n, self._head_shape(B, c), torch.float32)
        hp = (ctypes.c_void_p * len(self.head_names))(*[out[n].data_ptr() for n in self.head_names])
        with torch.cuda.device(self.device):
            rc = self.L.cp_forward(self.plan, B, _ptr(xs[0]), _ptr(xs[1]), _ptr(xs[2]), _ptr(xs[3]), hp, _stream())
        _lib.check(rc, "cp_forward")
        return out

    def profile(self, x, pre_img=None, pre_hm=None, pre_hm_hp=None):
        B, xs = self._check_inputs(x, pre_img, pre_hm, pre_hm_hp)
        out = {n: torch.empty(self._head_shape(B, c), dtype=torch.float32, device=self.device)
               for n, c in self.heads.items()}
        hp = (ctypes.c_void_p * len(self.head_names))(*[out[n].data_ptr() for n in self.head_names])
        n_ops = int(self.L.cp_plan_num_ops(self.plan))
        stats = (_lib.CpOpStat * n_ops)()
        n = ctypes.c_int32(0)
        with torch.cuda.device(self.device):
            rc = self.L.cp_plan_profile(self.plan, B, _ptr(xs[0]), _ptr(xs[1]), _ptr(xs[2]), _ptr(xs[3]), hp, _stream(),
                                        stats, n_ops, ctypes.byref(n))
        _lib.check(rc, "cp_plan_profile")
        return [dict(name=stats[i].name.decode(), kind=int(stats[i].kind), ms=float(stats[i].ms),
                     flops=float(stats[i].flops), bytes=float(stats[i].bytes)) for i in range(n.value)]

    @staticmethod
    def _act(a):
        return dict(off=int(a.off), ext=int(a.ext), C=int(a.C), H=int(a.H), W=int(a.W), stride=int(a.stride))

    def op_descs(self, model=0):
        out = []
        for i in range(int(self.L.cp_plan_num_ops(self.plan))):
            d = _lib.CpOpDesc()
            _lib.check(self.L.cp_plan_op_desc_model(self.plan, int(model), i, ctypes.byref(d)), "cp_plan_op_desc")
            r = {}
            for name, _ in _lib.CpOpDesc._fields_:
                v = getattr(d, name)
                if isinstance(v, _lib.CpActDesc):
                    v = self._act(v)
                elif name == "src":
                    v = [self._act(a) for a in v][:max(1, int(d.nsrc))]
                elif name == "children":
                    v = [int(c) for c in v][:int(d.n_children)]
                elif name == "name":
                    v = v.decode()
                elif v is None:
                    v = 0
                r[name] = v
            r["index"] = i
            out.append(r)
        return out

    def arena(self):
        p, n = ctypes.c_void_p(), ctypes.c_int64()
        _lib.check(self.L.cp_plan_arena(self.plan, ctypes.byref(p), ctypes.byref(n)), "cp_plan_arena")
        return _device_view(p.value, int(n.value), self.device)

    def run_ops(self, x, first, last, out, pre_img=None, pre_hm=None, pre_hm_hp=None):
        B, xs = self._check_inputs(x, pre_img, pre_hm, pre_hm_hp)
        for n, c in self.heads.items():
            self._out_tensor(out[n], "out[%s]" % n, self._head_shape(B, c), torch.float32)
        hp = (ctypes.c_void_p * len(self.head_names))(*[out[n].data_ptr() for n in self.head_names])
        n = max(0, last - first)
        info = (_lib.CpOpLaunch * max(1, n))()
        with torch.cuda.device(self.device):
            rc = self.L.cp_plan_run_ops(self.plan, B, first, last, _ptr(xs[0]), _ptr(xs[1]), _ptr(xs[2]), _ptr(xs[3]),
                                        hp, _stream(), info)
        _lib.check(rc, "cp_plan_run_ops")
        return [dict(family=int(info[i].family), BN=int(info[i].BN), ksplit=int(info[i].ksplit),
                     grid=int(info[i].grid)) for i in range(n)]

    def infer(self, x, meta, prm, pre_img=None, pre_hm=None, pre_hm_hp=None, heads_out=None, want_dets=False,
              poses=None, n_valid=None, dets=None):
        B, xs = self._check_inputs(x, pre_img, pre_hm, pre_hm_hp)
        lead = self._lead(B)
        if not torch.is_tensor(meta) or tuple(meta.shape) != (B, _lib.CP_META_DOUBLES):
            raise ValueError("meta must be a [%d,%d] tensor (make_meta)" % (B, _lib.CP_META_DOUBLES))
        if meta.device != self.device or meta.dtype != torch.float64 or not meta.is_contiguous():
            meta = meta.to(self.device, torch.float64).contiguous()
        if self.models > 1:
            prms = list(prm)
            if len(prms) != self.models:
                raise ValueError("a plan of %d models needs %d decode parameter sets, got %d" % (self.models, self.models,
                                                                                                len(prms)))
            K = prms[0].K
        else:
            K = prm.K
        if poses is None:
            poses = torch.empty(lead + (K, _lib.CP_POSE_RECORD), dtype=torch.float32, device=self.device)
        else:
            self._out_tensor(poses, "poses", lead + (K, _lib.CP_POSE_RECORD), torch.float32)
        if n_valid is None:
            n_valid = torch.empty(lead, dtype=torch.int32, device=self.device)
        else:
            self._out_tensor(n_valid, "n_valid", lead, torch.int32)
        if want_dets and dets is None:
            dets = torch.empty(lead + (K, _lib.CP_DETS_RECORD), dtype=torch.float32, device=self.device)
        elif dets is not None:
            self._out_tensor(dets, "dets", lead + (K, _lib.CP_DETS_RECORD), torch.float32)
        hp = None
        if heads_out is not None:
            for n, c in self.heads.items():
                self._out_tensor(heads_out[n], "heads_out[%s]" % n, self._head_shape(B, c), torch.float32)
            hp = (ctypes.c_void_p * len(self.head_names))(*[heads_out[n].data_ptr() for n in self.head_names])
        with torch.cuda.device(self.device):
            if self.models > 1 and self.tracking:
                arr = (_lib.CpDecodeParams * self.models)(*prms)
                rc = self.L.cp_infer_multi_track(self.plan, B, _ptr(xs[0]), _ptr(xs[1]), _ptr(xs[2]), _ptr(xs[3]), arr,
                                                 _ptr(meta), hp, _ptr(dets), _ptr(poses), _ptr(n_valid), _stream())
            elif self.models > 1:
                arr = (_lib.CpDecodeParams * self.models)(*prms)
                rc = self.L.cp_infer_multi(self.plan, B, _ptr(xs[0]), arr, _ptr(meta), hp, _ptr(dets), _ptr(poses),
                                           _ptr(n_valid), _stream())
            else:
                rc = self.L.cp_infer(self.plan, B, _ptr(xs[0]), _ptr(xs[1]), _ptr(xs[2]), _ptr(xs[3]), ctypes.byref(prm),
                                     _ptr(meta), hp, _ptr(dets), _ptr(poses), _ptr(n_valid), _stream())
        _lib.check(rc, ("cp_infer_multi_track" if self.tracking else "cp_infer_multi") if self.models > 1 else "cp_infer")
        return dets, poses, n_valid


class InferGraph(object):

    def __init__(self, eng, batch, prm, tracking=False):
        self.eng, self.prm = eng, prm
        dev = eng.device
        H, W = eng.height, eng.width
        self.x = torch.zeros((batch, 3, H, W), dtype=torch.float32, device=dev)
        self.meta = torch.zeros((batch, _lib.CP_META_DOUBLES), dtype=torch.float64, device=dev)
        self.meta[:, 2] = float(max(H, W))
        self.meta[:, 3], self.meta[:, 4] = W, H
        self.meta[:, 5], self.meta[:, 9], self.meta[:, 13] = 1.0, 1.0, 1.0
        self.pre = None
        if tracking:
            self.pre = (torch.zeros_like(self.x), torch.zeros((batch, 1, H, W), dtype=torch.float32, device=dev),
                        torch.zeros((batch, 8, H, W), dtype=torch.float32, device=dev))
        self.poses = torch.zeros((batch, prm.K, _lib.CP_POSE_RECORD), dtype=torch.float32, device=dev)
        self.n_valid = torch.zeros((batch,), dtype=torch.int32, device=dev)
        pre = self.pre if self.pre is not None else (None, None, None)
        side = torch.cuda.Stream(device=dev)
        side.wait_stream(torch.cuda.current_stream(dev))
        with torch.cuda.stream(side):
            for _ in range(2):
                eng.infer(self.x, self.meta, prm, *pre, poses=self.poses, n_valid=self.n_valid)
        torch.cuda.current_stream(dev).wait_stream(side)
        torch.cuda.synchronize(dev)
        self.graph = torch.cuda.CUDAGraph()
        with torch.cuda.graph(self.graph):
            eng.infer(self.x, self.meta, prm, *pre, poses=self.poses, n_valid=self.n_valid)

    def __call__(self, x, meta, pre_img=None, pre_hm=None, pre_hm_hp=None):
        self.x.copy_(x, non_blocking=True)
        self.meta.copy_(meta, non_blocking=True)
        if self.pre is not None:
            for dst, src in zip(self.pre, (pre_img, pre_hm, pre_hm_hp)):
                dst.copy_(src, non_blocking=True)
        self.graph.replay()
        return self.poses, self.n_valid


def preprocess(frames_u8, dst_h, dst_w, mean, std, out=None, trans_input=None):
    L = _lib.load()
    if not frames_u8.is_cuda or frames_u8.dtype != torch.uint8:
        raise RuntimeError("preprocess needs a uint8 CUDA tensor")
    B, sh, sw, _ = frames_u8.shape
    if out is None:
        out = torch.empty((B, 3, dst_h, dst_w), dtype=torch.float32, device=frames_u8.device)
    m = (ctypes.c_float * 3)(*[float(v) for v in mean])
    s = (ctypes.c_float * 3)(*[float(v) for v in std])
    with torch.cuda.device(frames_u8.device):
        if trans_input is not None:
            tm = (ctypes.c_double * 6)(*[float(v) for v in np.asarray(trans_input, np.float64).reshape(-1)])
            rc = L.cp_preprocess_affine(_ptr(frames_u8.contiguous()), _ptr(out), B, sh, sw, dst_h, dst_w, tm, m, s, _stream())
        else:
            rc = L.cp_preprocess(_ptr(frames_u8.contiguous()), _ptr(out), B, sh, sw, dst_h, dst_w, m, s, _stream())
    _lib.check(rc, "cp_preprocess")
    return out


def preprocess_ragged(packed_u8, offsets, src_hw, dst_h, dst_w, mean, std, out=None, trans_input=None):
    L = _lib.load()
    if not packed_u8.is_cuda or packed_u8.dtype != torch.uint8 or not packed_u8.is_contiguous():
        raise RuntimeError("preprocess_ragged needs a contiguous uint8 CUDA buffer")
    offs = np.ascontiguousarray(offsets, np.int64).reshape(-1)
    hw = np.ascontiguousarray(src_hw, np.int32).reshape(-1, 2)
    B = offs.shape[0]
    if hw.shape[0] != B:
        raise ValueError("preprocess_ragged: %d offsets for %d frame sizes" % (B, hw.shape[0]))
    if out is None:
        out = torch.empty((B, 3, dst_h, dst_w), dtype=torch.float32, device=packed_u8.device)
    tm = None
    if trans_input is not None:
        tr = np.ascontiguousarray(trans_input, np.float64).reshape(-1)
        if tr.shape[0] != 6 * B:
            raise ValueError("preprocess_ragged: trans_input must hold %d 2x3 matrices" % B)
        tm = tr.ctypes.data_as(ctypes.POINTER(ctypes.c_double))
    m = (ctypes.c_float * 3)(*[float(v) for v in mean])
    s = (ctypes.c_float * 3)(*[float(v) for v in std])
    with torch.cuda.device(packed_u8.device):
        rc = L.cp_preprocess_ragged(_ptr(packed_u8), packed_u8.numel(), offs.ctypes.data_as(ctypes.POINTER(ctypes.c_int64)),
                                    hw.ctypes.data_as(ctypes.POINTER(ctypes.c_int32)), _ptr(out), B, dst_h, dst_w, tm, m, s,
                                    _stream())
    _lib.check(rc, "cp_preprocess_ragged")
    return out


_YUV420 = {"nv12": _lib.CP_PIX_NV12, "i420": _lib.CP_PIX_I420}


def check_pixel_format(pixel_format):
    if pixel_format not in _lib.PIXEL_FORMATS:
        raise ValueError("pixel_format must be one of %s, got %r" % (", ".join(_lib.PIXEL_FORMATS), pixel_format))
    return pixel_format


def frame_shape(h, w, pixel_format):
    if check_pixel_format(pixel_format) == "bgr":
        return (int(h), int(w), 3)
    if h % 2 or w % 2 or h < 2 or w < 2:
        raise ValueError("%s frames need an even, positive image size; got %d x %d" % (pixel_format, h, w))
    return (int(h) * 3 // 2, int(w))


def image_size(shape, pixel_format, what="frame"):
# ... 99 lines not shown
```

### include/centerpose_b200.h

```cpp
#ifndef CENTERPOSE_B200_H_
#define CENTERPOSE_B200_H_

#include <stddef.h>
#include <stdint.h>

#ifdef __cplusplus
extern "C" {
#endif

#define CP_ABI_VERSION 1

enum cp_status {
  CP_OK = 0,
  CP_ERR_INVALID = -1,
  CP_ERR_CUDA = -2,
  CP_ERR_NOT_LOADED = -3,
  CP_ERR_MISSING_KEY = -4,
  CP_ERR_SHAPE = -5
};

enum cp_arch {
  CP_ARCH_DLA34 = 0,
  CP_ARCH_DLAV1_34 = 1,
  CP_ARCH_RES_18 = 2,
  CP_ARCH_RES_34 = 3,
  CP_ARCH_RES_50 = 4,
  CP_ARCH_RES_101 = 5,
  CP_ARCH_RES_152 = 6
};

enum cp_precision {
  CP_PREC_FP32 = 0,
  CP_PREC_TF32X3 = 1,
  CP_PREC_BF16 = 2,
  CP_PREC_TF32 = 3
};

#define CP_MAX_HEADS 16
#define CP_POSE_RECORD 192
#define CP_DETS_RECORD 128
#define CP_META_DOUBLES 16
#define CP_MAX_K 128
#define CP_MAX_CLASSES 80
#define CP_MAX_MODELS 16

typedef struct cp_plan cp_plan;

typedef struct cp_config {
  int32_t arch;
  int32_t tracking;
  int32_t tracking_task_gru;
  int32_t max_batch;
  int32_t height, width;
  int32_t precision;
  int32_t device;
  int32_t head_conv;
  int32_t num_heads;
  const char* head_names[CP_MAX_HEADS];
  int32_t head_channels[CP_MAX_HEADS];
} cp_config;

int cp_plan_create(const cp_config* cfg, cp_plan** out);
int cp_plan_destroy(cp_plan* plan);

int cp_plan_create_multi(const cp_config* cfg, int32_t num_models, cp_plan** out);
int cp_plan_create_multi_track(const cp_config* cfg, int32_t num_models, cp_plan** out);

#define CP_PLAN_REUSE_ACTIVATIONS 1u
#define CP_PLAN_MULTI_TRACK 2u
int cp_plan_create_ex(const cp_config* cfg, int32_t num_models, uint32_t flags, cp_plan** out);
typedef struct cp_memory_info {
  int64_t activation_bytes;
  int64_t weight_bytes;
  int64_t tile_bytes;
  int64_t workspace_bytes;
} cp_memory_info;
int cp_plan_memory(const cp_config* cfg, int32_t num_models, uint32_t flags, cp_memory_info* out);
typedef struct cp_act_alloc {
  int64_t floats;
  int64_t off;
  int32_t first, last;
} cp_act_alloc;
int cp_plan_allocations(const cp_config* cfg, int32_t num_models, uint32_t flags, cp_act_alloc* out, int32_t max_allocs,
                        int32_t* n_allocs);

int cp_plan_load_weights_model(cp_plan* plan, int32_t model, const char* const* names, const void* const* dev_ptrs,
                               const int64_t* numel, int32_t n, void* stream);
int32_t cp_plan_num_models(const cp_plan* plan);

int cp_plan_load_weights(cp_plan* plan, const char* const* names, const void* const* dev_ptrs,
                         const int64_t* numel, int32_t n, void* stream);

int cp_forward(cp_plan* plan, int32_t batch, const float* images, const float* pre_img,
               const float* pre_hm, const float* pre_hm_hp, float* const* head_out, void* stream);

typedef struct cp_op_stat {
  char name[96];
  int32_t kind;
  float ms;
  double flops;
  double bytes;
} cp_op_stat;
int cp_plan_num_ops(const cp_plan* plan);
int cp_plan_profile(cp_plan* plan, int32_t batch, const float* images, const float* pre_img,
                    const float* pre_hm, const float* pre_hm_hp, float* const* head_out, void* stream,
                    cp_op_stat* stats, int32_t max_stats, int32_t* n_stats);

enum cp_op_family {
  CP_FAM_NONE = 0,
  CP_FAM_IGEMM_FP32 = 1,
  CP_FAM_STEM = 2,
  CP_FAM_CONV3_C16 = 3,
  CP_FAM_IGEMM_UMMA = 4,
  CP_FAM_CONV_TMA = 5,
  CP_FAM_DCN_TMA = 6,
  CP_FAM_MAXPOOL = 7, CP_FAM_UPADD = 8, CP_FAM_GN_RELU = 9, CP_FAM_GRU = 10
};
typedef struct cp_act_desc {
  int64_t off;
  int32_t ext;
  int32_t C, H, W, stride;
} cp_act_desc;
typedef struct cp_op_desc {
  char name[96];
  int32_t kind;
  int32_t family;
  int32_t x3;
  int32_t nsrc;
  cp_act_desc src[4];
  cp_act_desc out;
  int32_t out_head;
  int32_t kh, stride, pad, Cin, Cout, CoutPad, Kpad;
  const float* w;
  int32_t w_ld;
  const float* bias;
  int32_t relu, has_res, res_after_relu;
  cp_act_desc res;
  cp_act_desc om;
  const float* up_w;
  int32_t f, has_skip;
  cp_act_desc skip;
  const float* gamma;
  const float* beta;
  int32_t groups;
  cp_act_desc gx, gh, gprev;
  int32_t first_step;
  int32_t fuse_heads;
  int32_t fused_away;
  int32_t parent;
  int32_t n_children;
  int32_t children[CP_MAX_HEADS];
} cp_op_desc;
typedef struct cp_op_launch {
  int32_t family;
  int32_t BN;
  int32_t ksplit;
  int32_t grid;
} cp_op_launch;
int cp_plan_op_desc(const cp_plan* plan, int32_t i, cp_op_desc* out);
int cp_plan_op_desc_model(const cp_plan* plan, int32_t model, int32_t i, cp_op_desc* out);
int cp_plan_arena(const cp_plan* plan, float** act, int64_t* floats);
int cp_plan_run_ops(cp_plan* plan, int32_t batch, int32_t first, int32_t last, const float* images, const float* pre_img,
                    const float* pre_hm, const float* pre_hm_hp, float* const* head_out, void* stream,
                    cp_op_launch* info);

int64_t cp_plan_bytes(const cp_plan* plan);
int32_t cp_plan_forward_launches(const cp_plan* plan);

typedef struct cp_heads {
  const float* hm;
  const float* wh;
  const float* hps;
  const float* reg;
  const float* hm_hp;
  const float* hp_offset;
  const float* scale;
  const float* hps_uncertainty;
  const float* scale_uncertainty;
  const float* tracking;
  const float* tracking_hp;
} cp_heads;

typedef struct cp_decode_params {
  int32_t batch, out_h, out_w;
  int32_t num_classes;
  int32_t num_joints;
  int32_t K;
  int32_t rep_mode;
  int32_t use_moments;
  int32_t nms;
  int32_t visible_thresh;
  int32_t opencv_return;
  int32_t apply_sigmoid;
  int32_t use_pnp;
  float vis_thresh;
  float balance;
  int32_t modern_bool_semantics;
  float test_scale;
  int32_t num_scales;
} cp_decode_params;

size_t cp_decode_workspace_bytes(const cp_decode_params* prm);
int cp_decode_pnp(const cp_decode_params* prm, const cp_heads* heads, const double* meta,
                  float* dets, float* poses, int32_t* n_valid,
                  void* workspace, size_t workspace_bytes, void* stream);

int cp_infer(cp_plan* plan, int32_t batch, const float* images, const float* pre_img,
             const float* pre_hm, const float* pre_hm_hp, const cp_decode_params* prm,
             const double* meta, float* const* heads_out, float* dets, float* poses,
             int32_t* n_valid, void* stream);

int cp_infer_multi(cp_plan* plan, int32_t batch, const float* images, const cp_decode_params* prms, const double* meta,
                   float* const* heads_out, float* dets, float* poses, int32_t* n_valid, void* stream);
int cp_infer_multi_track(cp_plan* plan, int32_t batch, const float* images, const float* pre_img, const float* pre_hm,
                         const float* pre_hm_hp, const cp_decode_params* prms, const double* meta, float* const* heads_out,
                         float* dets, float* poses, int32_t* n_valid, void* stream);

enum cp_pose_field {
  CP_P_SCORE = 0, CP_P_CLS = 1, CP_P_STATUS = 2, CP_P_NPTS = 3,
  CP_P_BBOX = 4,
  CP_P_CT = 8,
  CP_P_KPS = 10,
  CP_P_KPS_DISP_MEAN = 26,
  CP_P_KPS_HM_MEAN = 42,
  CP_P_KPS_HM_STD = 58,
  CP_P_KPS_HM_HEIGHT = 74,
  CP_P_KPS_DISP_STD = 82,
  CP_P_OBJ_SCALE = 98,
  CP_P_OBJ_SCALE_UNC = 101,
  CP_P_TRACKING = 104,
  CP_P_TRACKING_HP = 106,
  CP_P_LOCATION = 122,
  CP_P_QUAT = 125,
  CP_P_REPROJ = 129,
  CP_P_PROJ_CUBOID = 130,
  CP_P_KPS_3D_CAM = 146,
  CP_P_KPS_PNP = 173,
  CP_P_SRC_INDEX = 191
};

enum cp_pnp_status {
  CP_PNP_NOT_RUN = 0,
  CP_PNP_OK = 1,
  CP_PNP_INVISIBLE = 2,
  CP_PNP_BEHIND = 3,
  CP_PNP_FEW_POINTS = 4,
  CP_PNP_SOLVER_FAIL = 5
};

enum cp_dets_field {
  CP_D_BBOX = 0, CP_D_SCORE = 4, CP_D_CLS = 5,
  CP_D_KPS = 6,
  CP_D_OBJ_SCALE = 22,
  CP_D_OBJ_SCALE_UNC = 25,
  CP_D_TRACKING = 28,
  CP_D_TRACKING_HP = 30,
  CP_D_KPS_DISP_MEAN = 46,
  CP_D_KPS_DISP_STD = 62,
  CP_D_KPS_HM_MEAN = 78,
  CP_D_KPS_HM_STD = 94,
  CP_D_KPS_HM_HEIGHT = 110,
  CP_D_IND = 118
};

#define CP_TRACK_RECORD 320
typedef struct cp_tracker cp_tracker;
typedef struct cp_tracker_config {
  int32_t streams;
  int32_t max_tracks;
  int32_t kalman;
  int32_t scale_pool;
  int32_t use_pnp;
  int32_t hps_uncertainty;
  int32_t max_age;
  int32_t visible_thresh;
  int32_t opencv_return;
  int32_t render_hm_mode;
  int32_t render_hmhp_mode;
  int32_t device;
  float new_thresh;
  float pre_thresh;
  float R;
  float conf_lo, conf_hi;
  int32_t hungarian;
} cp_tracker_config;

int cp_tracker_create(const cp_tracker_config* cfg, cp_tracker** out);
int cp_tracker_create_multi(const cp_tracker_config* cfgs, int32_t models, cp_tracker** out);
int cp_tracker_destroy(cp_tracker* trk);
int cp_tracker_reset(cp_tracker* trk, int32_t index, void* stream);
int cp_tracker_step(cp_tracker* trk, int32_t batch, const float* poses, const int32_t* n_valid, int32_t K,
                    const double* meta, float* tracks_out, int32_t* n_tracks, void* stream);
int cp_tracker_step_ex(cp_tracker* trk, int32_t batch, const int32_t* stream_ids, const float* poses,
                       const int32_t* n_valid, int32_t K, const double* meta, float* tracks_out, int32_t* n_tracks,
                       void* stream);
int cp_tracker_render(cp_tracker* trk, int32_t batch, const double* meta, const double* trans_input, int32_t inp_h,
                      int32_t inp_w, float* pre_hm, float* pre_hm_hp, void* stream);
enum cp_render_mode {
  CP_RENDER_TRACKS = 0,
  CP_RENDER_GT = 1,
  CP_RENDER_EMPTY = 2
};
int cp_tracker_render_ex(cp_tracker* trk, int32_t batch, const double* meta, const double* trans_input, int32_t inp_h,
                         int32_t inp_w, const int32_t* modes, float* pre_hm, float* pre_hm_hp, void* stream);
int cp_tracker_render_ex2(cp_tracker* trk, int32_t batch, const int32_t* stream_ids, const double* meta,
                          const double* trans_input, int32_t inp_h, int32_t inp_w, const int32_t* modes, float* pre_hm,
                          float* pre_hm_hp, void* stream);

#define CP_SEED_RECORD 264
enum cp_seed_field {
// ... 68 lines not shown
```

Before: 678.3.

## Add 2-D spatial tiles and decoupled K-chunk pipelining to TMA conv

Adds a 2-D tiling mode for 3x3 TMA convolutions. Each tile covers 2 rows by 64 columns, so the halo slab is 4x66 rather than several full padded rows. This shrinks each A slab and lets the x3 path keep 32-channel slabs, consumed in 16- or 32-wide K chunks (kch) separate from the slab width. The MMA loop also stops waiting on every wgmma and waits only at group ends, deferring barrier releases so tensor-core work overlaps. The cost is added indexing complexity, a changed split-K heuristic, and correctness risk in the deferred release logic.

New measurement: 700.2 (median of 6 runs). 1.03x the previous value.

```diff
diff --git a/centerpose_b200/_lib.py b/centerpose_b200/_lib.py
--- a/centerpose_b200/_lib.py
+++ b/centerpose_b200/_lib.py
@@ -87,7 +87,7 @@
 
 
 class CpOpLaunch(ctypes.Structure):
-    _fields_ = [(n, ctypes.c_int32) for n in ("family", "BN", "ksplit", "grid")]
+    _fields_ = [(n, ctypes.c_int32) for n in ("family", "BN", "ksplit", "grid", "cslab", "tile2d")]
 
 
 class CpMemoryInfo(ctypes.Structure):
diff --git a/centerpose_b200/csrc/common.cuh b/centerpose_b200/csrc/common.cuh
--- a/centerpose_b200/csrc/common.cuh
+++ b/centerpose_b200/csrc/common.cuh
@@ -81,6 +81,8 @@
   int BN = 0;
   int ksplit = 1;
   long long grid = 0;
+  int cslab = 0;
+  int tile2d = 0;
 };
 
 bool conv3_c16_supported(const IgemmParams& p);
@@ -95,6 +97,8 @@
   int BN = 0;
   int cslab = 0;
   size_t wbytes = 0;
+  bool tile2d = false;
+  int kch = 0;
 };
 struct ConvPolicy {
   bool small_on_cuda_cores;
@@ -153,12 +157,13 @@
 bool tma_conv_supported(const IgemmParams& p, int x3);
 size_t tma_weight_bytes(int Cin, int taps, int CoutPad, int x3);
 int tma_tile_n(int CoutPad, int x3);
-int tma_cslab(const IgemmParams& p, int x3);
+bool tma_tile2d(const IgemmParams& p);
+int tma_cslab(const IgemmParams& p, int x3, bool tile2d);
 int launch_pack_tma_weight(const float* src_k_by_ld, int ld, int Cin, int taps, int Cout, int CoutPad, int x3, int cslab,
                            int bn, void* dst, cudaStream_t s);
 int tma_encode_nhwc_box(const float* base, int C, int W, int H, int B, int strideFloats, int boxC, int boxW, int boxH,
                         int swizzle64, void* map_out );
-int tma_conv_encode(const IgemmParams& p, int Bmax, int cslab, void* maps_out );
+int tma_conv_encode(const IgemmParams& p, int Bmax, int cslab, bool tile2d, void* maps_out );
 int launch_conv_tma(const IgemmParams& p, const void* maps, const ConvKernel& k, cudaStream_t stream, LaunchInfo* info);
 
 bool dcn_tma_supported(const IgemmParams& p, int x3);
diff --git a/centerpose_b200/csrc/conv_select.cu b/centerpose_b200/csrc/conv_select.cu
--- a/centerpose_b200/csrc/conv_select.cu
+++ b/centerpose_b200/csrc/conv_select.cu
@@ -4,17 +4,32 @@
 
 namespace cp {
 
+static bool env_on(const char* name) {
+  const char* e = getenv(name);
+  return e && atoi(e) != 0;
+}
+
+static ConvKernel conv_tma_kernel_of(const IgemmParams& p, bool x3, bool round_out) {
+  ConvKernel k{CP_FAM_CONV_TMA, x3, round_out, tma_tile_n(p.CoutPad, x3), 0,
+               tma_weight_bytes(p.Cin, p.kh * p.kw, p.CoutPad, x3)};
+  k.tile2d = tma_tile2d(p) && !env_on("CP_CONV_TMA_FLAT");
+  k.cslab = tma_cslab(p, x3, k.tile2d);
+  k.kch = tma_cslab(p, x3, false);
+  return k;
+}
+
 ConvKernel select_conv_kernel(const IgemmParams& p, int32_t precision, const ConvPolicy& pol) {
   const bool small = p.mode == IGEMM_NCHW_SCALAR || p.Cin < 32;
   if (precision != CP_PREC_FP32 && !(pol.small_on_cuda_cores && small)) {
     const bool tma = precision == CP_PREC_TF32 || precision == CP_PREC_TF32X3;
     const bool x3 = precision == CP_PREC_TF32X3;
-    if (tma && pol.dcn_tma && dcn_tma_supported(p, x3))
-      return {CP_FAM_DCN_TMA, x3, pol.round_out && !x3, dcn_tma_tile_n(p.CoutPad, x3), 16,
-              tma_weight_bytes(p.Cin, 9, p.CoutPad, x3)};
-    if (tma && tma_conv_supported(p, x3))
-      return {CP_FAM_CONV_TMA, x3, pol.round_out && !x3, tma_tile_n(p.CoutPad, x3), tma_cslab(p, x3),
-              tma_weight_bytes(p.Cin, p.kh * p.kw, p.CoutPad, x3)};
+    if (tma && pol.dcn_tma && dcn_tma_supported(p, x3)) {
+      ConvKernel k{CP_FAM_DCN_TMA, x3, pol.round_out && !x3, dcn_tma_tile_n(p.CoutPad, x3), 16,
+                   tma_weight_bytes(p.Cin, 9, p.CoutPad, x3)};
+      k.kch = 16;
+      return k;
+    }
+    if (tma && tma_conv_supported(p, x3)) return conv_tma_kernel_of(p, x3, pol.round_out && !x3);
     const bool gx3 = gather_x3(precision);
     const int phases = p.mode == IGEMM_DECONV ? 4 : 1;
     if (umma_supported(p, gx3))
@@ -27,7 +42,7 @@
 
 int conv_encode(const ConvKernel& k, const IgemmParams& p, int Bmax, TmaMaps* maps) {
   if (k.family == CP_FAM_DCN_TMA) return dcn_tma_encode(p, Bmax, maps->map);
-  if (k.family == CP_FAM_CONV_TMA) return tma_conv_encode(p, Bmax, k.cslab, maps->map);
+  if (k.family == CP_FAM_CONV_TMA) return tma_conv_encode(p, Bmax, k.cslab, k.tile2d, maps->map);
   return CP_OK;
 }
 
@@ -35,7 +50,7 @@
   switch (k.family) {
     case CP_FAM_DCN_TMA:
     case CP_FAM_CONV_TMA:
-      return launch_pack_tma_weight(p.wgt, ld, p.Cin, p.kh * p.kw, p.Cout, p.CoutPad, k.x3, k.cslab, k.BN, tiles, s);
+      return launch_pack_tma_weight(p.wgt, ld, p.Cin, p.kh * p.kw, p.Cout, p.CoutPad, k.x3, k.kch, k.BN, tiles, s);
     case CP_FAM_IGEMM_UMMA: {
       const int phases = p.mode == IGEMM_DECONV ? 4 : 1;
       const size_t phase_bytes = k.wbytes / phases;
diff --git a/centerpose_b200/csrc/conv_tma.cu b/centerpose_b200/csrc/conv_tma.cu
--- a/centerpose_b200/csrc/conv_tma.cu
+++ b/centerpose_b200/csrc/conv_tma.cu
@@ -7,6 +7,7 @@
 namespace {
 
 constexpr int TM_BM = 128;
+constexpr int TM_TW = 64;
 constexpr int TM_THREADS = 384;
 constexpr int TM_THREADS_X3 = 512;
 
@@ -18,6 +19,8 @@
   int k;
   int tile_m;
   int Wt, boxh;
+  int tile2d;
+  int tiles_x;
   int tiles_per_image;
   long long total_tiles;
   long long m_tiles;
@@ -30,6 +33,7 @@
   int outStride, out_nchw;
   int round_tf32;
   int cslab;
+  int kch;
   int x3;
   int group;
   const unsigned char* wtiles;
@@ -53,7 +57,7 @@
 static_assert(sizeof(TmaCtl) <= 512, "control block");
 
 struct TileGeo {
-  int n_tile, img, g0, r_lo, model;
+  int n_tile, img, g0, ax, ay, row0, model;
   long long pos0;
 };
 template <bool MULTI>
@@ -63,14 +67,24 @@
   const long long m_tile = ct / n_tiles;
   g.img = 0;
   g.g0 = 0;
-  g.r_lo = 0;
+  g.ax = g.ay = g.row0 = 0;
   g.pos0 = 0;
   g.model = 0;
   if (p.k == 3) {
     g.img = (int)(m_tile / p.tiles_per_image);
-    g.g0 = (int)(m_tile - (long long)g.img * p.tiles_per_image) * p.tile_m;
-    const int t = g.g0 - 1;
-    g.r_lo = (t >= 0) ? t / p.Wt : -((-t + p.Wt - 1) / p.Wt);
+    const int t_img = (int)(m_tile - (long long)g.img * p.tiles_per_image);
+    if (p.tile2d) {
+      const int ty = t_img / p.tiles_x;
+      g.ax = (t_img - ty * p.tiles_x) * TM_TW - 1;
+      g.ay = 2 * ty - 1;
+    } else {
+      g.g0 = t_img * p.tile_m;
+      const int t = g.g0 - 1;
+      const int r_lo = (t >= 0) ? t / p.Wt : -((-t + p.Wt - 1) / p.Wt);
+      g.ax = -1;
+      g.ay = r_lo - 1;
+      g.row0 = t - r_lo * p.Wt;
+    }
     if (MULTI) g.model = g.img / p.ipm;
   } else if (MULTI) {
     g.model = (int)(m_tile / p.tiles_per_model);
@@ -84,7 +98,12 @@
 template <bool MULTI>
 __device__ __forceinline__ bool tile_position(const TmaConvParams& p, const TileGeo& g, int i, int* n, int* oy, int* ox, int* m) {
   bool valid;
-  if (p.k == 3) {
+  if (p.k == 3 && p.tile2d) {
+    *oy = g.ay + 1 + i / TM_TW;
+    *ox = g.ax + 1 + i % TM_TW;
+    *n = g.img;
+    valid = *oy < p.H;
+  } else if (p.k == 3) {
     const int gg = g.g0 + i;
     *oy = gg / p.Wt;
     const int xp = gg - *oy * p.Wt;
@@ -111,7 +130,7 @@
   if (threadIdx.x == 0) griddep_launch_dependents();
   const uint32_t slabs0 = (smem_u32(smem) + 512u + 1023u) & ~1023u;
   const uint32_t rowb = (uint32_t)p.cslab * 4u;
-  const uint32_t btile_bytes = (uint32_t)BN * rowb * (X3 ? 2u : 1u);
+  const uint32_t btile_bytes = (uint32_t)BN * p.kch * 4u * (X3 ? 2u : 1u);
   const uint32_t a_stage = p.slab_stride * (X3 ? 2u : 1u);
   const uint32_t btiles0 = slabs0 + (uint32_t)p.SA * a_stage;
   const uint32_t drain0 = btiles0 + (uint32_t)p.SB * btile_bytes;
@@ -121,8 +140,9 @@
   const int taps = p.k * p.k;
   const int KS_SPLIT = p.ksplit;
   const int sps = p.sps;
+  const int halves = p.cslab / p.kch;
   const int KB = sps * taps;
-  const int KB_all = (p.Cin / p.cslab) * taps;
+  const int KB_all = (p.Cin / p.kch) * taps;
   const long long total_tiles = p.total_tiles;
   const long long tph = FUSE ? p.tph : 1;
   auto tile_at = [&](long long it) { return ((long long)blockIdx.x + (it / tph) * gridDim.x) * tph + (it % tph); };
@@ -152,8 +172,10 @@
           const TileGeo g = decode_tile<MULTI>(p, tile / KS_SPLIT, n_tiles);
           const int s_begin = (int)(tile % KS_SPLIT) * sps;
           for (int s = s_begin; s < s_begin + sps; ++s) {
+            if (s != s_begin && s % halves) continue;
+            const int c0 = s / halves * p.cslab;
             int src = 0, cb = 0;
-            while (src + 1 < p.nsrc && s * p.cslab >= cb + p.srcC[src]) {
+            while (src + 1 < p.nsrc && c0 >= cb + p.srcC[src]) {
               cb += p.srcC[src];
               ++src;
             }
@@ -162,9 +184,9 @@
             mbar_arrive_expect_tx(bar, p.slab_bytes);
             const uint32_t dst = slabs0 + (uint32_t)stage * a_stage;
             if (p.k == 3)
-              tma_load_4d(dst, &p.amap[src], s * p.cslab - cb, -1, g.r_lo - 1, g.img, bar);
+              tma_load_4d(dst, &p.amap[src], c0 - cb, g.ax, g.ay, g.img, bar);
             else
-              tma_load_2d(dst, &p.amap[src], s * p.cslab - cb, (int)g.pos0, bar);
+              tma_load_2d(dst, &p.amap[src], c0 - cb, (int)g.pos0, bar);
             if (++stage == p.SA) {
               stage = 0;
               phase ^= 1u;
@@ -208,7 +230,9 @@
     uint32_t phase = 0;
     const uint32_t nchunk = p.slab_bytes >> 4;
     for (long long it = 0, tile = tile_at(0); tile < total_tiles; tile = tile_at(++it)) {
-      for (int s = 0; s < sps; ++s) {
+      const int s_begin = (int)(tile % KS_SPLIT) * sps;
+      const int n_slabs = (s_begin + sps - 1) / halves - s_begin / halves + 1;
+      for (int s = 0; s < n_slabs; ++s) {
         mbar_wait(smem_u32(&ctl->a_full[stage]), phase);
         const uint32_t hi = slabs0 + (uint32_t)stage * a_stage;
         const uint32_t lo = hi + p.slab_stride;
@@ -245,7 +269,7 @@
     const uint32_t bar_a = smem_u32(X3 ? &ctl->a_split[0] : &ctl->a_full[0]);
     const uint32_t bar_a_empty = smem_u32(&ctl->a_empty[0]);
     const uint32_t bar_b_full = smem_u32(&ctl->b_full[0]), bar_b_empty = smem_u32(&ctl->b_empty[0]);
-    const uint32_t a_lo_u = p.slab_stride >> 4, b_lo_u = ((uint32_t)BN * rowb) >> 4;
+    const uint32_t a_lo_u = p.slab_stride >> 4, b_lo_u = ((uint32_t)BN * p.kch * 4u) >> 4;
     EpiParams ep;
     ep.bias = p.bias;
     ep.residual = p.residual;
@@ -271,47 +295,61 @@
     for (int j = 0; j < (FUSE ? 16 : 1); ++j) acc2[j] = 0.f;
     for (long long it = 0, tile = tile_at(0); tile < total_tiles; tile = tile_at(++it)) {
       const TileGeo g = decode_tile<MULTI>(p, tile / KS_SPLIT, n_tiles);
-      const uint32_t row0 = (p.k == 3 ? (uint32_t)(g.g0 - 1 - g.r_lo * p.Wt) : 0u) + (uint32_t)c * 64u;
+      const uint32_t row0 = (uint32_t)g.row0 + (uint32_t)c * (p.tile2d ? (uint32_t)p.Wt : 64u);
 #pragma unroll
       for (int j = 0; j < (X3 ? BN / 2 : 1); ++j) sums[j] = 0.f;
       int kbi = 0, gk = 0;
-      for (int s = 0; s < sps; ++s) {
-        mbar_wait(bar_a + 8u * (uint32_t)sa, pa);
+      static_assert(kX3GroupBlocks == 1, "a group is at most two K blocks: one chained, one waited for");
+      int sb_held = -1, sa_held = -1;
+      const int s_begin = (int)(tile % KS_SPLIT) * sps, s_end = s_begin + sps;
+      for (int s = s_begin; s < s_end; ++s) {
+        const int h = s % halves;
+        if (s == s_begin || h == 0) mbar_wait(bar_a + 8u * (uint32_t)sa, pa);
+        const bool slab_done = h == halves - 1 || s == s_end - 1;
         const uint32_t a_slab = slabs0 + (uint32_t)sa * a_stage;
         for (int tap = 0; tap < taps; ++tap, ++kbi) {
           const int ky = tap / 3, kx = tap - ky * 3;
           const uint32_t arow = row0 + (p.k == 3 ? (uint32_t)(ky * p.Wt + kx) : 0u);
           mbar_wait(bar_b_full + 8u * (uint32_t)sb, pb);
-          const uint64_t da = make_desc(a_slab + arow * rowb, p.cslab);
-          const uint64_t db = make_desc(btiles0 + (uint32_t)sb * btile_bytes, p.cslab);
+          const uint64_t da = make_desc(a_slab + arow * rowb, p.cslab) + (uint64_t)(h * p.kch / 4);
+          const uint64_t db = make_desc(btiles0 + (uint32_t)sb * btile_bytes, p.kch);
           const bool fresh = X3 ? gk == 0 : kbi == 0;
-          if (p.cslab == 32)
-            mma_kblock<BN, X3, false, 4>(acc, da, db, a_lo_u, b_lo_u, fresh);
+          const bool group_end = !X3 || gk == p.group - 1 || kbi == KB - 1;
+          const bool releases_slab = tap == taps - 1 && slab_done;
+          const bool wait = group_end || (releases_slab && p.SA < 2);
+          if (p.kch == 32)
+            mma_kblock<BN, X3, false, 4>(acc, da, db, a_lo_u, b_lo_u, fresh, false);
           else
-            mma_kblock<BN, X3, false, 2>(acc, da, db, a_lo_u, b_lo_u, fresh);
-          if (wt == 0) {
-            mbar_arrive(bar_b_empty + 8u * (uint32_t)sb);
-            if (tap == taps - 1) mbar_arrive(bar_a_empty + 8u * (uint32_t)sa);
+            mma_kblock<BN, X3, false, 2>(acc, da, db, a_lo_u, b_lo_u, fresh, false);
+          if (wait) {
+            wg_wait<0>();
+            if (wt == 0) {
+              if (sb_held >= 0) mbar_arrive(bar_b_empty + 8u * (uint32_t)sb_held);
+              if (sa_held >= 0) mbar_arrive(bar_a_empty + 8u * (uint32_t)sa_held);
+              mbar_arrive(bar_b_empty + 8u * (uint32_t)sb);
+              if (releases_slab) mbar_arrive(bar_a_empty + 8u * (uint32_t)sa);
+            }
+            sb_held = sa_held = -1;
+            if (X3 && group_end) {
+#pragma unroll
+              for (int j = 0; j < (X3 ? BN / 2 : 1); ++j) sums[j] += acc[X3 ? j : 0];
+            }
+          } else {
+            sb_held = sb;
+            if (releases_slab) sa_held = sa;
           }
+          gk = group_end ? 0 : gk + 1;
           if (++sb == p.SB) {
             sb = 0;
             pb ^= 1u;
           }
-          if (X3) {
-            if (gk == p.group - 1 || kbi == KB - 1) {
-#pragma unroll
-              for (int j = 0; j < (X3 ? BN / 2 : 1); ++j) sums[j] += acc[X3 ? j : 0];
-              gk = 0;
-            } else {
-              ++gk;
-            }
-          }
         }
-        if (++sa == p.SA) {
+        if (slab_done && ++sa == p.SA) {
           sa = 0;
           pa ^= 1u;
         }
       }
+      wg_wait<0>();
       const int r_me = wt >> 1;
       int n, oy, ox, m;
       const bool valid = tile_position<MULTI>(p, g, c * 64 + r_me, &n, &oy, &ox, &m);
@@ -459,12 +497,18 @@
   return CP_OK;
 }
 
-int tma_cslab(const IgemmParams& p, int x3) {
+bool tma_tile2d(const IgemmParams& p) { return p.kh == 3 && p.Win % TM_TW == 0; }
+
+static int tma_slab_pitch(int W, bool tile2d) { return tile2d ? TM_TW + 2 : W + 2; }
+static int tma_slab_rows(int W, bool tile2d) { return tile2d ? 4 : tma_boxh(W + 2); }
+
+int tma_cslab(const IgemmParams& p, int x3, bool tile2d) {
   if (p.Cin % 32) return 16;
   if (!x3 || p.kh != 3) return 32;
-  const int Wt = p.Win + 2;
-  const int boxh = tma_boxh(Wt);
-  const size_t slab32 = ((size_t)boxh * Wt * 128 + 1023) / 1024 * 1024;
+  if (tile2d)
+    for (int s = 0; s < p.nsrc; ++s)
+      if (p.srcC[s] % 32) return 16;
+  const size_t slab32 = ((size_t)tma_slab_rows(p.Win, tile2d) * tma_slab_pitch(p.Win, tile2d) * 128 + 1023) / 1024 * 1024;
   const int bn = tma_tile_n(p.CoutPad, x3);
   const size_t need = 2 * (2 * slab32) + 2 * ((size_t)bn * 128 * 2);
   return need > TM_BUDGET ? 16 : 32;
@@ -476,7 +520,7 @@
   if (p.mode != IGEMM_NHWC_VEC) return false;
   if (!((p.kh == 1 && p.kw == 1 && p.pad == 0) || (p.kh == 3 && p.kw == 3 && p.pad == 1))) return false;
   if (p.stride != 1) return false;
-  const int cs = tma_cslab(p, x3);
+  const int cs = tma_cslab(p, x3, false);
   if (p.Cin % cs) return false;
   for (int s = 0; s < p.nsrc; ++s)
     if (p.srcC[s] % cs || p.srcStride[s] % 4) return false;
@@ -520,12 +564,12 @@
   return CP_OK;
 }
 
-int tma_conv_encode(const IgemmParams& p, int Bmax, int cs, void* maps_out) {
+int tma_conv_encode(const IgemmParams& p, int Bmax, int cs, bool tile2d, void* maps_out) {
   EncodeTiledFn enc = get_encode();
   if (!enc) return fail(CP_ERR_CUDA, "cuTensorMapEncodeTiled entry point not available");
   CUtensorMap* maps = reinterpret_cast<CUtensorMap*>(maps_out);
-  const int Wt = p.Win + 2;
-  const int boxh = tma_boxh(Wt);
+  const int Wt = tma_slab_pitch(p.Win, tile2d);
+  const int boxh = tma_slab_rows(p.Win, tile2d);
   const CUtensorMapSwizzle swz = cs == 32 ? CU_TENSOR_MAP_SWIZZLE_128B : CU_TENSOR_MAP_SWIZZLE_64B;
   for (int s = 0; s < p.nsrc; ++s) {
     CUresult r;
@@ -583,6 +627,7 @@
   if (!p.wgt_umma) return fail(CP_ERR_INVALID, "conv_tma: weight tiles missing");
   if (p.B % model_ipm(p)) return fail(CP_ERR_INVALID, "conv_tma: batch is not a whole number of models");
   const bool x3 = k.x3;
+  if (k.tile2d && !tma_tile2d(p)) return fail(CP_ERR_INVALID, "conv_tma: 2-D tiles need a 3x3 conv over a multiple of 64 columns");
   TmaConvParams q;
   memset(&q, 0, sizeof(q));
   memcpy(q.amap, maps, sizeof(CUtensorMap) * 4);
@@ -597,17 +642,21 @@
   q.BN = k.BN;
   q.x3 = x3;
   q.cslab = k.cslab;
-  q.group = kX3GroupBlocks * (32 / q.cslab);
+  q.kch = k.kch;
+  if ((q.kch != 16 && q.kch != 32) || q.cslab % q.kch) return fail(CP_ERR_INVALID, "conv_tma: K blocks must divide the slab");
+  q.group = kX3GroupBlocks * (32 / q.kch);
   q.k = p.kh;
-  q.Wt = p.Win + 2;
+  q.tile2d = k.tile2d;
+  q.Wt = tma_slab_pitch(p.Win, k.tile2d);
   q.tile_m = TM_BM;
-  q.boxh = tma_boxh(q.Wt);
+  q.boxh = tma_slab_rows(p.Win, k.tile2d);
   q.ipm = model_ipm(p);
   q.wstride = p.wstride;
   q.tstride = p.tstride;
   size_t m_tiles;
   if (q.k == 3) {
-    q.tiles_per_image = (p.Hin * q.Wt + q.tile_m - 1) / q.tile_m;
+    q.tiles_x = p.Win / TM_TW;
+    q.tiles_per_image = k.tile2d ? (p.Hin + 1) / 2 * q.tiles_x : (p.Hin * q.Wt + q.tile_m - 1) / q.tile_m;
     m_tiles = (size_t)q.tiles_per_image * p.B;
     q.slab_bytes = (uint32_t)q.boxh * q.Wt * (uint32_t)q.cslab * 4u;
   } else {
@@ -617,7 +666,7 @@
     q.slab_bytes = (uint32_t)q.tile_m * (uint32_t)q.cslab * 4u;
   }
   q.slab_stride = (q.slab_bytes + 1023u) & ~1023u;
-  const uint32_t btile = (uint32_t)q.BN * (uint32_t)q.cslab * 4u * (x3 ? 2u : 1u);
+  const uint32_t btile = (uint32_t)q.BN * (uint32_t)q.kch * 4u * (x3 ? 2u : 1u);
   const uint32_t a_stage = q.slab_stride * (x3 ? 2u : 1u);
   size_t smem = 0;
   if (int rc = tma_smem_layout(a_stage, btile, q.k, &q.SA, &q.SB, &smem)) return rc;
@@ -646,10 +695,14 @@
   q.m_tiles = (long long)m_tiles;
   q.part = p.splitk_ws;
   const long long mn = (long long)m_tiles * (p.CoutPad / q.BN);
-  const int nslab = q.Cin / q.cslab;
+  const int nslab = q.Cin / q.kch;
   int num_sms = 0;
   if (int rc = device_sm_count(&num_sms)) return rc;
-  q.ksplit = x3 && !q.fuse ? splitk_factor(mn, nslab, num_sms, (size_t)q.tile_m * q.BN, p.splitk_ws_floats) : 1;
+  const long long mn_flat = q.tile2d ? (long long)((p.Hin * (p.Win + 2) + q.tile_m - 1) / q.tile_m) * p.B * (p.CoutPad / q.BN)
+                                     : mn;
+  q.ksplit = x3 && !q.fuse ? splitk_factor(mn_flat, nslab, num_sms, (size_t)q.tile_m * q.BN, p.splitk_ws_floats) : 1;
+  if (q.ksplit > 1 && (size_t)mn * q.ksplit * q.tile_m * q.BN > p.splitk_ws_floats)
+    return fail(CP_ERR_INVALID, "conv_tma: split-K workspace too small");
   q.sps = nslab / q.ksplit;
   q.total_tiles = mn * q.ksplit;
   if (q.total_tiles >= (1ll << 31)) return fail(CP_ERR_INVALID, "conv_tma: too many tiles");
@@ -671,6 +724,8 @@
     info->BN = q.BN;
     info->ksplit = q.ksplit;
     info->grid = cfg.gridDim.x;
+    info->cslab = q.cslab;
+    info->tile2d = q.tile2d;
   }
   if (q.ksplit > 1) {
     const long long threads = mn * (q.BN / 4) * q.tile_m;
diff --git a/centerpose_b200/csrc/dcn_tma.cu b/centerpose_b200/csrc/dcn_tma.cu
--- a/centerpose_b200/csrc/dcn_tma.cu
+++ b/centerpose_b200/csrc/dcn_tma.cu
@@ -517,6 +517,7 @@
     info->BN = q.BN;
     info->ksplit = q.ksplit;
     info->grid = grid;
+    info->cslab = k.cslab;
   }
   if (q.ksplit > 1) {
     const long long threads = mn * (q.BN / 4) * DT_BM;
diff --git a/centerpose_b200/csrc/plan.cu b/centerpose_b200/csrc/plan.cu
--- a/centerpose_b200/csrc/plan.cu
+++ b/centerpose_b200/csrc/plan.cu
@@ -1018,6 +1018,8 @@
       li.BN = tc.BN;
       li.ksplit = tc.ksplit;
       li.grid = (int32_t)tc.grid;
+      li.cslab = tc.cslab;
+      li.tile2d = tc.tile2d;
       break;
     }
     case OP_MAXPOOL:
diff --git a/centerpose_b200/csrc/umma_common.cuh b/centerpose_b200/csrc/umma_common.cuh
--- a/centerpose_b200/csrc/umma_common.cuh
+++ b/centerpose_b200/csrc/umma_common.cuh
@@ -161,7 +161,7 @@
 
 template <int BN, bool X3, bool BF16, int KS>
 __device__ __forceinline__ void mma_kblock(float (&acc)[BN / 2], uint64_t da, uint64_t db, uint32_t a_lo, uint32_t b_lo,
-                                           bool fresh) {
+                                           bool fresh, bool wait = true) {
   wg_fence();
 #pragma unroll
   for (int ks = 0; ks < KS; ++ks) {
@@ -180,7 +180,7 @@
     for (int ks = 0; ks < KS; ++ks) wgmma_tf32<BN>(acc, da + 2u * ks, db + 2u * ks, 1u);
   }
   wg_commit();
-  wg_wait<0>();
+  if (wait) wg_wait<0>();
 }
 
 __device__ __forceinline__ float tf32_round(float x) {
diff --git a/centerpose_b200/engine.py b/centerpose_b200/engine.py
--- a/centerpose_b200/engine.py
+++ b/centerpose_b200/engine.py
@@ -322,7 +322,7 @@
                                         hp, _stream(), info)
         _lib.check(rc, "cp_plan_run_ops")
         return [dict(family=int(info[i].family), BN=int(info[i].BN), ksplit=int(info[i].ksplit),
-                     grid=int(info[i].grid)) for i in range(n)]
+                     grid=int(info[i].grid), cslab=int(info[i].cslab), tile2d=int(info[i].tile2d)) for i in range(n)]
 
     def infer(self, x, meta, prm, pre_img=None, pre_hm=None, pre_hm_hp=None, heads_out=None, want_dets=False,
               poses=None, n_valid=None, dets=None):
diff --git a/include/centerpose_b200.h b/include/centerpose_b200.h
--- a/include/centerpose_b200.h
+++ b/include/centerpose_b200.h
@@ -156,6 +156,8 @@
   int32_t BN;
   int32_t ksplit;
   int32_t grid;
+  int32_t cslab;
+  int32_t tile2d;
 } cp_op_launch;
 int cp_plan_op_desc(const cp_plan* plan, int32_t i, cp_op_desc* out);
 int cp_plan_op_desc_model(const cp_plan* plan, int32_t model, int32_t i, cp_op_desc* out);
```
